# shubhamchandak94/HARC

Measured on AMD Instinct MI355X. Metric: Mreads/s reorder+encode, 100 bp, higher is better.
Workload: dtype u64 (2-bit packed bases, XOR+popcount)

## Files before the change

harc_amd/api.py:

```python
import ctypes as C
import os

HERE = os.path.dirname(os.path.abspath(__file__))


class HarcAmdError(RuntimeError):
    def __init__(self, code, msg):
        super().__init__(f"harc_amd error {code}: {msg}")
        self.code = code


class Params(C.Structure):
    _fields_ = [("readlen", C.c_int32), ("num_thr", C.c_int32), ("num_chains", C.c_int32), ("maxmatch", C.c_int32),
                ("thresh", C.c_int32), ("thresh_s", C.c_int32), ("maxsearch", C.c_int32), ("dict_start", C.c_int32 * 2),
                ("dict_end", C.c_int32 * 2), ("device", C.c_int32), ("profile", C.c_int32), ("num_steps", C.c_int32), ("reads_per_chain", C.c_int32), ("decode_memory_gb", C.c_int32), ("stream_digest", C.c_int32), ("table_slots_per_read", C.c_int32)]


class Counters(C.Structure):
    _fields_ = [("n_clean", C.c_uint64), ("n_N", C.c_uint64), ("n_main", C.c_uint64), ("n_singleton", C.c_uint64),
                ("unmatched", C.c_uint64), ("aligned_singletons", C.c_uint64), ("aligned_N", C.c_uint64),
                ("chains", C.c_uint64), ("rounds", C.c_uint64), ("probes", C.c_uint64), ("candidates", C.c_uint64),
                ("conflicts", C.c_uint64), ("propose_launches", C.c_uint64), ("propose_ms", C.c_double),
                ("index_ms", C.c_double), ("chain_ms", C.c_double), ("encode_ms", C.c_double), ("total_ms", C.c_double),
                ("contigs", C.c_uint64), ("seq_bases", C.c_uint64), ("bins_over_maxsearch", C.c_uint64),
# ... 48 lines not shown
    l.harc_amd_set_reads_ascii.argtypes = [ctx, C.c_char_p, C.c_uint32, C.c_uint32]
    l.harc_amd_set_reads_ascii_device.argtypes = [ctx, C.c_void_p, C.c_uint32, C.c_uint32]
    l.harc_amd_set_reads_packed_device.argtypes = [ctx, C.c_void_p, C.c_uint32]
    l.harc_amd_set_nreads_ascii.argtypes = [ctx, C.c_char_p, C.c_uint32, C.c_uint32]
    l.harc_amd_set_nreads_ascii_device.argtypes = [ctx, C.c_void_p, C.c_uint32, C.c_uint32]
    l.harc_amd_set_stage1_streams.argtypes = [ctx, C.c_char_p, C.c_char_p, C.c_char_p, C.c_char_p, C.c_char_p, C.c_uint32,
                                              C.c_char_p, C.c_char_p, C.c_uint32]
    l.harc_amd_pack_reads_device.argtypes = [ctx, C.c_void_p, C.c_uint32, C.c_uint32, C.c_void_p]
    l.harc_amd_bucket_reads_device.argtypes = [ctx, C.c_void_p, C.c_uint32, C.c_uint32, C.c_void_p]
    l.harc_amd_partition_reads_device.argtypes = [ctx, C.c_void_p, C.c_uint32, C.c_uint32, C.c_void_p, C.c_void_p]
    for f in ("harc_amd_reorder", "harc_amd_encode", "harc_amd_pack_order"):
        getattr(l, f).argtypes = [ctx]
    l.harc_amd_get_stream.argtypes = [ctx, C.c_int32, C.c_int32, C.POINTER(C.c_void_p), C.POINTER(C.c_size_t)]
    l.harc_amd_get_counters.argtypes = [ctx, C.POINTER(Counters)]
    for f in ("harc_amd_reorder_files", "harc_amd_encoder_files", "harc_amd_compress_files", "harc_amd_pack_order_files"):
        getattr(l, f).argtypes = [PP, C.c_char_p]
    l.harc_amd_preprocess_files.argtypes = [C.c_char_p, C.c_char_p, C.c_int32]
    l.harc_amd_decoder_files.argtypes = [PP, C.c_char_p, C.c_int32]
    l.harc_amd_compress_fastq_files_ex.argtypes = [PP, C.c_char_p, C.c_char_p, C.c_int32, C.c_int32]
    l.harc_amd_build_has.argtypes = [C.c_char_p]
    l.harc_amd_last_fastq_timing.argtypes = [C.POINTER(C.c_double), C.c_int32]
    l.harc_amd_decoder_preserve_files.argtypes = [PP, C.c_char_p, C.c_int32]
    l.harc_amd_compress_fastq_files.argtypes = [PP, C.c_char_p, C.c_char_p]
    l.harc_amd_set_fastq_device.argtypes = [ctx, C.c_void_p, C.c_uint64, C.POINTER(C.c_uint64)]
    l.harc_amd_bgzf_inflate_device.argtypes = [ctx, C.c_void_p, C.c_uint64, C.c_void_p, C.c_uint64, C.POINTER(C.c_uint64)]
    l.harc_amd_set_fastq_bgzf_device.argtypes = [ctx, C.c_void_p, C.c_uint64, C.POINTER(C.c_uint64)]
    l.harc_amd_fastq_assemble_device.argtypes = [ctx, C.c_void_p, C.c_uint64, C.c_void_p, C.c_void_p, C.c_uint32, C.c_int32, C.c_void_p, C.c_uint64,
                                                 C.POINTER(C.c_uint64)]
    l.harc_amd_fastq_assemble_files.argtypes = [PP, C.c_char_p, C.c_char_p, C.c_char_p, C.c_char_p]
    l.harc_amd_fastq_assemble_files_ex.argtypes = [PP, C.c_char_p, C.c_char_p, C.c_char_p, C.c_char_p, C.c_int32]
    l.harc_amd_bgzf_bound.argtypes = [C.c_uint64]
    l.harc_amd_bgzf_bound.restype = C.c_uint64
    l.harc_amd_bgzf_deflate_device.argtypes = [ctx, C.c_void_p, C.c_uint64, C.c_int32, C.c_void_p, C.c_uint64, C.POINTER(C.c_uint64)]
    l.harc_amd_bgzf_deflate_host.argtypes = [C.c_char_p, C.c_uint64, C.c_int32, C.c_char_p, C.c_uint64, C.POINTER(C.c_uint64)]
    l.harc_amd_qpack_bound.argtypes = [C.c_uint64, C.c_int32, C.c_uint32]
    l.harc_amd_qpack_bound.restype = C.c_uint64
    l.harc_amd_qpack_device.argtypes = [ctx, C.c_void_p, C.c_uint64, C.c_int32, C.c_uint32, C.c_int32, C.c_void_p, C.c_uint64, C.POINTER(C.c_uint64)]
    l.harc_amd_qunpack_device.argtypes = [ctx, C.c_void_p, C.c_uint64, C.c_void_p, C.c_uint64, C.POINTER(C.c_uint64)]
    l.harc_amd_qpack_host.argtypes = [C.c_char_p, C.c_uint64, C.c_int32, C.c_uint32, C.c_int32, C.c_char_p, C.c_uint64, C.POINTER(C.c_uint64)]
    l.harc_amd_qunpack_host.argtypes = [C.c_char_p, C.c_uint64, C.c_char_p, C.c_uint64, C.POINTER(C.c_uint64)]
    l.harc_amd_qpack_files.argtypes = [PP, C.c_char_p, C.c_char_p]
    l.harc_amd_qunpack_files.argtypes = [PP, C.c_char_p, C.c_char_p]
    QM, QS = C.POINTER(QMap), C.POINTER(QMapStats)
    l.harc_amd_qmap_parse.argtypes = [C.c_char_p, QM]
    l.harc_amd_qmap_host.argtypes = [C.c_char_p, C.c_uint64, C.c_int32, QM, C.c_char_p, QS]
    l.harc_amd_qmap_device.argtypes = [ctx, C.c_void_p, C.c_uint64, C.c_int32, QM, C.c_void_p, QS]
    l.harc_amd_qmap_files.argtypes = [PP, C.c_char_p, C.c_char_p, QM, QS]
    l.harc_amd_qpack_files_ex.argtypes = [PP, C.c_char_p, C.c_char_p, QM, QS]
    l.harc_amd_idpack_bound.argtypes = [C.c_uint64, C.c_uint64, C.c_uint32]
    l.harc_amd_idpack_bound.restype = C.c_uint64
    l.harc_amd_idpack_device.argtypes = [ctx, C.c_void_p, C.c_uint64, C.c_uint32, C.c_int32, C.c_void_p, C.c_uint64, C.POINTER(C.c_uint64)]
    l.harc_amd_idunpack_device.argtypes = [ctx, C.c_void_p, C.c_uint64, C.c_void_p, C.c_uint64, C.POINTER(C.c_uint64)]
    l.harc_amd_idpack_host.argtypes = [C.c_char_p, C.c_uint64, C.c_uint32, C.c_int32, C.c_char_p, C.c_uint64, C.POINTER(C.c_uint64)]
    l.harc_amd_idunpack_host.argtypes = [C.c_char_p, C.c_uint64, C.c_char_p, C.c_uint64, C.POINTER(C.c_uint64)]
    l.harc_amd_idpack_files.argtypes = [PP, C.c_char_p, C.c_char_p]
    l.harc_amd_idunpack_files.argtypes = [PP, C.c_char_p, C.c_char_p]
    l.harc_amd_spack_bound.argtypes = [C.c_uint64, C.c_uint32]
    l.harc_amd_spack_bound.restype = C.c_uint64
    l.harc_amd_spack_device.argtypes = [ctx, C.c_void_p, C.c_uint64, C.c_uint32, C.c_int32, C.c_void_p, C.c_uint64, C.POINTER(C.c_uint64)]
    l.harc_amd_sunpack_device.argtypes = [ctx, C.c_void_p, C.c_uint64, C.c_void_p, C.c_uint64, C.POINTER(C.c_uint64)]
    l.harc_amd_spack_host.argtypes = [C.c_char_p, C.c_uint64, C.c_uint32, C.c_int32, C.c_char_p, C.c_uint64, C.POINTER(C.c_uint64)]
    l.harc_amd_sunpack_host.argtypes = [C.c_char_p, C.c_uint64, C.c_char_p, C.c_uint64, C.POINTER(C.c_uint64)]
    l.harc_amd_spack_files.argtypes = [PP, C.c_char_p, C.c_char_p]
    l.harc_amd_sunpack_files.argtypes = [PP, C.c_char_p, C.c_char_p]
    l.harc_amd_spack_file_list.argtypes = [PP, C.c_int32, C.POINTER(C.c_char_p), C.POINTER(C.c_char_p)]
    l.harc_amd_sunpack_file_list.argtypes = [PP, C.c_int32, C.POINTER(C.c_char_p), C.POINTER(C.c_char_p)]
    l.harc_amd_decode_signature.argtypes = [ctx, C.POINTER(C.c_uint64)]
    l.harc_amd_input_signature.argtypes = [ctx, C.POINTER(C.c_uint64)]
    l.harc_amd_reads_signature_device.argtypes = [ctx, C.c_void_p, C.c_uint32, C.c_uint32, C.POINTER(C.c_uint64)]
    l.harc_amd_comm_get_id.argtypes = [C.c_char_p, C.c_size_t]
    l.harc_amd_comm_init.argtypes = [ctx, C.c_char_p, C.c_size_t, C.c_int32, C.c_int32]
    l.harc_amd_comm_init_mailbox.argtypes = [ctx, C.c_char_p, C.c_int32, C.c_int32]
    l.harc_amd_comm_barrier.argtypes = [ctx]
    l.harc_amd_comm_destroy.argtypes = [ctx]
    l.harc_amd_shard_exchange.argtypes = [ctx, C.POINTER(C.c_uint64)]
    l.harc_amd_shard_reset.argtypes = [ctx]
    l.harc_amd_replicate_exchange.argtypes = [ctx, C.POINTER(C.c_uint64)]
    l.harc_amd_compress_fastq_shard_files.argtypes = [PP, C.c_char_p, C.c_char_p, C.c_int32, C.c_int32, C.c_int32, C.c_int32, C.c_char_p]
    l.harc_amd_merge_shard_files.argtypes = [C.c_char_p, C.c_int32]
    l.harc_amd_stream_digest.argtypes = [ctx, C.POINTER(C.c_uint64)]
    l.harc_amd_selftest_launch.argtypes = [ctx, C.c_uint64, C.POINTER(C.c_uint64), C.POINTER(C.c_uint64)]
    l.harc_amd_selftest_index.argtypes = [ctx, C.c_void_p, C.c_uint64, C.c_int32, C.c_uint32, C.c_int32, C.POINTER(C.c_uint64), C.POINTER(C.c_uint32), C.c_void_p, C.c_void_p,
                                          C.c_void_p, C.c_uint64, C.POINTER(C.c_uint64)]
    U3 = C.POINTER(C.c_uint64)
    l.harc_amd_text_digest_device.argtypes = [ctx, C.c_void_p, C.c_uint64, C.c_uint64, U3]
    l.harc_amd_text_digest_host.argtypes = [C.c_char_p, C.c_uint64, C.c_uint64, U3]
    l.harc_amd_text_digest_files.argtypes = [PP, C.c_char_p, U3]
    l.harc_amd_input_order_digest.argtypes = [ctx, U3]
    l.harc_amd_reads_check_files.argtypes = [PP, C.c_char_p, U3, U3]
    l.harc_amd_compress_fastq_files_checked.argtypes = [PP, C.c_char_p, C.c_char_p, C.c_int32, C.c_int32, C.c_int32]
    l.harc_amd_build_id.restype = C.c_char_p
    _lib = l
    return l


def _check(rc):
    if rc != 0:
        raise HarcAmdError(rc, lib().harc_amd_last_error().decode(errors="replace"))


def default_params(readlen, num_thr=8, num_chains=0, device=0, profile=0, num_steps=0, reads_per_chain=0, stream_digest=0, table_slots_per_read=0):
    p = Params()
    _check(lib().harc_amd_default_params(readlen, C.byref(p)))
    p.num_thr, p.num_chains, p.device, p.profile, p.num_steps = num_thr, num_chains, device, profile, num_steps
    p.reads_per_chain = reads_per_chain
    p.stream_digest = stream_digest
    p.table_slots_per_read = table_slots_per_read
    return p


def build_id():
    return lib().harc_amd_build_id().decode()


def reorder(basedir, readlen, num_chains=1, **kw):
    p = default_params(readlen, num_chains=num_chains, **kw)
    _check(lib().harc_amd_reorder_files(C.byref(p), os.fsencode(basedir)))


def encoder(basedir, readlen, num_thr=1, **kw):
    p = default_params(readlen, num_thr=num_thr, **kw)
    _check(lib().harc_amd_encoder_files(C.byref(p), os.fsencode(basedir)))


def compress(basedir, readlen, num_thr=1, num_chains=1, **kw):
    p = default_params(readlen, num_thr=num_thr, num_chains=num_chains, **kw)
    _check(lib().harc_amd_compress_files(C.byref(p), os.fsencode(basedir)))


def preprocess(fastq, basedir, readlen):
    _check(lib().harc_amd_preprocess_files(os.fsencode(fastq), os.fsencode(basedir), readlen))


def compress_fastq(fastq, basedir, readlen, num_thr=1, num_chains=1, preserve_order=False, preserve_quality=False, check=False, **kw):
    p = default_params(readlen, num_thr=num_thr, num_chains=num_chains, **kw)
    _check(lib().harc_amd_compress_fastq_files_checked(C.byref(p), os.fsencode(fastq), os.fsencode(basedir), int(preserve_order), int(preserve_quality), int(check)))


def build_has(feature):
    return bool(lib().harc_amd_build_has(feature.encode()))


def last_fastq_timing(n=8):
    t = (C.c_double * n)()
    _check(lib().harc_amd_last_fastq_timing(t, n))
    names = ("context_and_pool", "ingest", "ingest_waiting_for_file_readers", "ingest_device_passes", "reorder", "encode", "stream_files", "total",
             "ingest_bgzf_inflate")
    return {k: float(v) for k, v in zip(names, t)}


COMM_ID_BYTES = 128


def comm_get_id():
    b = C.create_string_buffer(COMM_ID_BYTES)
    _check(lib().harc_amd_comm_get_id(b, COMM_ID_BYTES))
    return b.raw


def compress_fastq_shard(fastq, basedir, readlen, world, rank, comm_spec, num_thr=1, num_chains=0, preserve_order=False,
                         preserve_quality=False, **kw):
    kw.setdefault("reads_per_chain", 1024)
    p = default_params(readlen, num_thr=num_thr, num_chains=num_chains, **kw)
    _check(lib().harc_amd_compress_fastq_shard_files(C.byref(p), os.fsencode(fastq), os.fsencode(basedir), int(preserve_order),
                                                     int(preserve_quality), world, rank, os.fsencode(comm_spec)))

# ... 312 lines not shown
        _check(lib().harc_amd_comm_init(self._ctx, comm_id, len(comm_id), world, rank))

    def comm_init_mailbox(self, directory, world, rank):
        _check(lib().harc_amd_comm_init_mailbox(self._ctx, os.fsencode(directory), world, rank))

    def comm_barrier(self):
        _check(lib().harc_amd_comm_barrier(self._ctx))

    def comm_destroy(self):
        _check(lib().harc_amd_comm_destroy(self._ctx))

    def shard_exchange(self):
        info = (C.c_uint64 * 8)()
        _check(lib().harc_amd_shard_exchange(self._ctx, info))
        return tuple(int(x) for x in info)

    def replicate_exchange(self):
        info = (C.c_uint64 * 8)()
        _check(lib().harc_amd_replicate_exchange(self._ctx, info))
        return tuple(int(x) for x in info)

    def shard_reset(self):
        _check(lib().harc_amd_shard_reset(self._ctx))

    def reorder(self):
        _check(lib().harc_amd_reorder(self._ctx))

    def encode(self):
        _check(lib().harc_amd_encode(self._ctx))

    def pack_order(self):
        _check(lib().harc_amd_pack_order(self._ctx))

    def decode_signature(self):
        sig = (C.c_uint64 * 3)()
        _check(lib().harc_amd_decode_signature(self._ctx, sig))
        return tuple(int(x) for x in sig)

    def input_signature(self):
        sig = (C.c_uint64 * 3)()
        _check(lib().harc_amd_input_signature(self._ctx, sig))
        return tuple(int(x) for x in sig)

    def text_digest_device(self, ptr, nbytes, first_offset=0, acc=(0, 0, 0)):
        a = (C.c_uint64 * 3)(*acc)
        _check(lib().harc_amd_text_digest_device(self._ctx, C.c_void_p(ptr) if ptr else None, nbytes, first_offset, a))
        return tuple(a)

    def input_order_digest(self):
        a = (C.c_uint64 * 3)()
        _check(lib().harc_amd_input_order_digest(self._ctx, a))
        return tuple(a)

    def reads_signature_device(self, d_ascii, n, stride):
        sig = (C.c_uint64 * 3)()
        _check(lib().harc_amd_reads_signature_device(self._ctx, C.c_void_p(d_ascii), n, stride, sig))
        return tuple(int(x) for x in sig)

    def stream(self, name, shard=0):
        ptr, ln = C.c_void_p(), C.c_size_t()
        _check(lib().harc_amd_get_stream(self._ctx, STREAMS[name], shard, C.byref(ptr), C.byref(ln)))
        return C.string_at(ptr, ln.value) if ln.value else b""

    def selftest_launch(self, n):
        v, x = C.c_uint64(0), C.c_uint64(0)
        _check(lib().harc_amd_selftest_launch(self._ctx, n, C.byref(v), C.byref(x)))
        return int(v.value), int(x.value)

    def selftest_index(self, keys, slots_per_read=0, bigthresh=0, want_large=False):
        import numpy as np
        keys = np.ascontiguousarray(keys, dtype=np.uint64)
        n = int(keys.size)
        cap, nbins, nl = C.c_uint64(0), C.c_uint32(0), C.c_uint64(0)
        _check(lib().harc_amd_selftest_index(self._ctx, keys.ctypes.data, n, slots_per_read, bigthresh, 0, C.byref(cap), None, None, None, None, 0, None))
        slots = np.zeros(cap.value, dtype=np.dtype([("key", "<u8"), ("start", "<u4"), ("count", "<u4")]))
        ids = np.zeros(n, dtype=np.uint32)
        large = np.zeros(n // 16 + 16, dtype=np.uint64)
        _check(lib().harc_amd_selftest_index(self._ctx, keys.ctypes.data, n, slots_per_read, bigthresh, 1 if want_large else 0, C.byref(cap), C.byref(nbins),
                                             slots.ctypes.data, ids.ctypes.data, large.ctypes.data, large.size, C.byref(nl)))
        if want_large and nl.value > large.size:
            raise HarcAmdError(-1, "harc_amd_selftest_index lists %d large bins among %d keys" % (nl.value, n))
        return int(cap.value), int(nbins.value), slots, ids, (large[:nl.value].copy() if want_large else None)

    def stream_digest(self):
        d = (C.c_uint64 * 4)()
        _check(lib().harc_amd_stream_digest(self._ctx, d))
        return tuple(int(x) for x in d)

    def counters(self):
        c = Counters()
        _check(lib().harc_amd_get_counters(self._ctx, C.byref(c)))
        return c
```

harc_amd/csrc/api.cpp:

```cpp
#include "internal.h"
#include <stdarg.h>
#include <chrono>
#include <stdlib.h>

static thread_local char g_err[512] = "";
void harc_set_error(const char *fmt, ...)
{
    va_list ap; va_start(ap, fmt); vsnprintf(g_err, sizeof g_err, fmt, ap); va_end(ap);
}
extern "C" const char *harc_amd_last_error(void) { return g_err; }

static size_t pool_hand_back(harc_amd_ctx *c, size_t from, size_t asked)
{
    size_t given = 0;
    for (size_t i = 0; i < c->pool.size(); i++) {
        harc_amd_ctx::PoolChunk &k = c->pool[i];
        if (i == from || k.size == 0 || k.used != 0) continue;
        (void)hipFree(k.base); c->pool_total -= k.size; given += k.size; k.base = nullptr; k.size = 0;
    }
    if (given) {
        (void)hipGetLastError();
        if (getenv("HARC_AMD_TRACE")) fprintf(stderr, "[pool] %.2f GB of empty chunks handed back for a request of %.2f GB\n", given / 1e9, asked / 1e9);
    }
    return given;
}
int harc_raw_alloc(harc_amd_ctx *c, void **p, size_t bytes)
{
    *p = nullptr;
    if (bytes == 0) bytes = 16;
    hipError_t e = hipMalloc(p, bytes);
    if (e != hipSuccess) (void)hipGetLastError();
    if (e != hipSuccess && !c->pool.empty() && pool_hand_back(c, c->pool_cur, bytes)) e = hipMalloc(p, bytes);
    if (e != hipSuccess) { (void)hipGetLastError(); harc_set_error("hipMalloc(%zu) failed: %s", bytes, hipGetErrorString(e)); return HARC_AMD_ENOMEM; }
    c->owned.push_back(*p);
    c->sizes[*p] = bytes;
    c->dev_bytes += bytes;
    if (c->dev_bytes > c->dev_peak) c->dev_peak = c->dev_bytes;
    return HARC_AMD_OK;
}
void harc_raw_free(harc_amd_ctx *c, void *p)
{
    if (!p) return;
    for (size_t i = 0; i < c->owned.size(); i++)
        if (c->owned[i] == p) { c->owned[i] = c->owned.back(); c->owned.pop_back(); break; }
    auto it = c->sizes.find(p);
    if (it != c->sizes.end()) { c->dev_bytes -= it->second; c->sizes.erase(it); }
    (void)hipFree(p);
}
static size_t pool_in_use(const harc_amd_ctx *c)
{
    size_t u = 0;
    for (size_t i = 0; i <= c->pool_cur && i < c->pool.size(); i++) u += c->pool[i].used;
    return u;
}
int harc_dev_alloc(harc_amd_ctx *c, void **p, size_t bytes)
{
    *p = nullptr;
    if (const char *e = getenv("HARC_AMD_FAIL_ALLOC")) {
        static long long countdown = -1;
        if (countdown < 0) countdown = atoll(e);
        if (countdown > 0 && --countdown == 0) { harc_set_error("pool allocation refused (HARC_AMD_FAIL_ALLOC)"); return HARC_AMD_ENOMEM; }
    }
    bytes = (bytes + 255) & ~(size_t)255;
    if (bytes == 0) bytes = 256;
    const size_t cur_in = c->pool_cur;
    for (;;) {
        if (c->pool_cur < c->pool.size()) {
            harc_amd_ctx::PoolChunk &k = c->pool[c->pool_cur];
            if (k.used + bytes <= k.size) { *p = k.base + k.used; k.used += bytes; break; }
            if (c->pool_cur + 1 < c->pool.size()) { c->pool_cur++; c->pool[c->pool_cur].used = 0; continue; }
        }
        size_t want = bytes;
        const size_t grow = c->pool_total < ((size_t)8 << 30) ? c->pool_total : ((size_t)8 << 30);
        if (want < grow / 2) want = grow;
        if (want < ((size_t)64 << 20)) want = (size_t)64 << 20;
        void *base = nullptr;
        hipError_t e = hipMalloc(&base, want);
        if (e != hipSuccess) (void)hipGetLastError();
        if (e != hipSuccess && want > bytes) { want = bytes; e = hipMalloc(&base, want); if (e != hipSuccess) (void)hipGetLastError(); }
        if (e != hipSuccess && !c->pool.empty() && pool_hand_back(c, cur_in, bytes)) e = hipMalloc(&base, want);
        if (e != hipSuccess) { (void)hipGetLastError(); harc_set_error("hipMalloc(%zu) failed: %s", want, hipGetErrorString(e)); return HARC_AMD_ENOMEM; }
        if (getenv("HARC_AMD_POISON")) (void)hipMemset(base, 0xA5, want);
        if (getenv("HARC_AMD_TRACE")) fprintf(stderr, "[pool] chunk %zu: %.2f GB for a request of %.2f GB (pool %.2f GB, in use %.2f GB)\n", c->pool.size(), want / 1e9, bytes / 1e9, (c->pool_total + want) / 1e9, pool_in_use(c) / 1e9);
        c->pool.push_back({ (char *)base, want, 0 });
        c->pool_total += want;
        c->pool_cur = c->pool.size() - 1;
    }
    const size_t live = c->dev_bytes + pool_in_use(c);
    if (live > c->dev_peak) c->dev_peak = live;
    return HARC_AMD_OK;
}
void harc_dev_free(harc_amd_ctx *c, void *p) { (void)c; (void)p; }
harc_mark_t harc_pool_mark(harc_amd_ctx *c)
{
    if (c->pool.empty()) return 0;
    return ((harc_mark_t)c->pool_cur << 48) | (harc_mark_t)c->pool[c->pool_cur].used;
}
void harc_pool_release(harc_amd_ctx *c, harc_mark_t m)
{
    if (c->pool.empty()) return;
    const size_t cur = (size_t)(m >> 48), used = (size_t)(m & (((harc_mark_t)1 << 48) - 1));
    for (size_t i = cur + 1; i < c->pool.size(); i++) c->pool[i].used = 0;
    c->pool[cur].used = used;
    c->pool_cur = cur;
}
int harc_host_alloc(harc_amd_ctx *c, void **p, size_t bytes)
{
    bytes = (bytes + 63) & ~(size_t)63;
    if (bytes == 0) bytes = 64;
    for (auto &k : c->harena) if (k.used + bytes <= k.size) { *p = k.base + k.used; k.used += bytes; return HARC_AMD_OK; }
    size_t want = bytes < ((size_t)16 << 20) ? ((size_t)16 << 20) : bytes + (bytes >> 2);
    void *base = nullptr;
    hipError_t e = hipHostMalloc(&base, want, hipHostMallocDefault);
    if (e != hipSuccess) { harc_set_error("hipHostMalloc(%zu) failed: %s", want, hipGetErrorString(e)); return HARC_AMD_ENOMEM; }
    c->harena.push_back({ (char *)base, want, bytes });
    *p = base;
    return HARC_AMD_OK;
}
void harc_host_reset(harc_amd_ctx *c) { for (auto &k : c->harena) k.used = 0; }
int harc_d2h(harc_amd_ctx *c, std::vector<uint8_t> &dst, const void *d_src, size_t bytes)
{
    dst.resize(bytes);
    if (bytes) HIP_TRY(hipMemcpyAsync(dst.data(), d_src, bytes, hipMemcpyDeviceToHost, c->stream));
    return HARC_AMD_OK;
}

extern "C" int harc_amd_default_params(int32_t L, harc_amd_params *p)
{
    if (!p || L < 1 || L > 255) { harc_set_error("readlen %d out of range 1..255 (harc:46-49; 256 breaks the pos byte, decoder.cpp:93)", L); return HARC_AMD_EINVAL; }
    memset(p, 0, sizeof *p);
    p->readlen = L; p->num_thr = 8; p->num_chains = 0;
    p->maxmatch = L / 2; p->thresh = 4; p->thresh_s = 24; p->maxsearch = 1000;
    const int h = L / 2;
    if (L > 100) { p->dict_start[0] = h - 32; p->dict_end[0] = h - 1; p->dict_start[1] = h; p->dict_end[1] = h - 1 + 32; }
    else { p->dict_start[0] = h - L * 32 / 100; p->dict_end[0] = h - 1; p->dict_start[1] = h; p->dict_end[1] = h - 1 + L * 32 / 100; }
    return HARC_AMD_OK;
}

static int check_params(const harc_amd_params *p)
{
    if (!p) return HARC_AMD_EINVAL;
    const int L = p->readlen;
    if (L < 1 || L > 255) { harc_set_error("readlen %d out of range 1..255", L); return HARC_AMD_EINVAL; }
    if (p->num_thr < 1 || p->num_thr > 4096) { harc_set_error("num_thr %d out of range", p->num_thr); return HARC_AMD_EINVAL; }
    if (p->num_chains < 0) { harc_set_error("num_chains < 0"); return HARC_AMD_EINVAL; }
    if (p->num_steps < 0 || p->num_steps > 64) { harc_set_error("num_steps %d out of range 0..64", p->num_steps); return HARC_AMD_EINVAL; }
    if (p->maxmatch < 0 || p->maxmatch > 128 || p->maxmatch > L) { harc_set_error("maxmatch out of range"); return HARC_AMD_EINVAL; }
    if (p->maxsearch < 1 || p->thresh < 0 || p->thresh_s < 0) { harc_set_error("thresholds out of range"); return HARC_AMD_EINVAL; }
    for (int l = 0; l < 2; l++) {
        const int n = p->dict_end[l] - p->dict_start[l] + 1;
        if (p->dict_start[l] < 0 || p->dict_end[l] >= L || n < 0 || n > 32) { harc_set_error("dictionary window %d out of range", l); return HARC_AMD_EINVAL; }
    }
    return HARC_AMD_OK;
}

extern "C" int harc_amd_create(const harc_amd_params *params, harc_amd_ctx **out)
{
    if (!out) return HARC_AMD_EINVAL;
    *out = nullptr;
    RC_TRY(check_params(params));
    int ndev = 0;
    hipError_t e = hipGetDeviceCount(&ndev);
    if (e != hipSuccess || ndev <= 0) { harc_set_error("no HIP device (%s); libharc_amd has no CPU fallback", e == hipSuccess ? "count=0" : hipGetErrorString(e)); return HARC_AMD_ENODEVICE; }
    if (params->device < 0 || params->device >= ndev) { harc_set_error("device %d not in [0,%d)", params->device, ndev); return HARC_AMD_EINVAL; }
    HIP_TRY(hipSetDevice(params->device));
    harc_amd_ctx *c = new harc_amd_ctx();
    c->P = *params;
    c->W = (2 * params->readlen + 63) / 64;
    c->W3 = (3 * params->readlen + 63) / 64;
    memset(&c->C, 0, sizeof c->C);
    if (hipStreamCreateWithFlags(&c->stream, hipStreamNonBlocking) != hipSuccess) { delete c; harc_set_error("hipStreamCreate failed"); return HARC_AMD_ENODEVICE; }
    if (hipStreamCreateWithFlags(&c->copy_stream, hipStreamNonBlocking) != hipSuccess || hipEventCreateWithFlags(&c->ev_copy, hipEventDisableTiming) != hipSuccess) {
        if (c->copy_stream) (void)hipStreamDestroy(c->copy_stream);
        (void)hipStreamDestroy(c->stream); delete c; harc_set_error("hipStreamCreate failed"); return HARC_AMD_ENODEVICE;
    }
// ... 312 lines not shown
```

harc_amd/csrc/internal.h:

```cpp
#pragma once
#include <hip/hip_runtime.h>
#include <stdint.h>
#include <stdio.h>
#include <string.h>
#include <map>
#include <string>
#include <utility>
#include <vector>
#include "../../include/harc_amd.h"

#define HARC_NONE 0xFFFFFFFFu
#define HARC_MAXW 8
#define HARC_MAXW3 12
#define HARC_MAXK (1u << 20)
#define HARC_LOOK_CHUNKS 16
#ifndef HARC_NSUGG
#define HARC_NSUGG 8
#endif

void harc_set_error(const char *fmt, ...);

#define HIP_TRY(expr)                                                                                          \
    do {                                                                                                       \
        hipError_t _e = (expr);                                                                                \
// ... 38 lines not shown
};
#define SLOT_DEAD 0x80000000u
#define SLOT_EMB 0x40000000u
#define SLOT_BIG 0x20000000u
#define SLOT_OVF 0x10000000u
#define SLOT_CNT_MASK 0x0FFFFFFFu

struct DictDev {
    HashSlot *slots = nullptr;
    uint64_t cap = 0;
    uint32_t *ids = nullptr;
    uint32_t *d_nbins = nullptr;
    uint32_t nbins = 0;
    unsigned long long *large_list = nullptr; unsigned int *large_n = nullptr; uint32_t large_max = 0, large_tag = 0;
    uint32_t bigthresh = 0;
};

struct harc_amd_ctx {
    harc_amd_params P;
    int W = 0, W3 = 0;
    hipStream_t stream = nullptr;
    hipStream_t copy_stream = nullptr;
    hipEvent_t ev_copy = nullptr;
    uint32_t s2_events_hint = 0;
    uint64_t s1_seq_key = 0; int s1_seq_choice = -1;
    size_t dev_bytes = 0, dev_peak = 0;
    std::vector<void *> owned;
    std::map<void *, size_t> sizes;
    struct PoolChunk { char *base; size_t size, used; };
    std::vector<PoolChunk> pool;
    size_t pool_cur = 0, pool_total = 0;

    uint32_t N = 0;  uint64_t *d_reads = nullptr;
    uint32_t NN = 0; uint64_t *d_nreads3 = nullptr;
    struct InBuf { void *p = nullptr; size_t cap = 0; };
    InBuf own_reads, own_nreads3;
    uint32_t N_own = 0, NN_own = 0;
    uint64_t nrec_own = 0;
    struct HarcComm *comm = nullptr;
    InBuf x_reads, x_nreads3, x_gid, x_ngid;
    uint32_t *d_gid = nullptr, *d_ngid = nullptr;
    int s2_world = 1, s2_rank = 0;
    bool s2_part = false; int s2_e0 = 0, s2_e1 = 0;
    bool replicated = false;
    uint64_t shard_info[8] = { 0, 0, 0, 0, 0, 0, 0, 0 };
    bool have_s1 = false;
    uint32_t M = 0, S = 0;
    uint32_t *d_order = nullptr; uint8_t *d_flag = nullptr, *d_pos = nullptr, *d_rc = nullptr; uint32_t *d_order_s = nullptr;
    uint64_t *d_oreads = nullptr;
    uint64_t *d_sreads = nullptr;
    bool s1_from_files = false;
    bool have_s2 = false;
    uint32_t *d_s2_order = nullptr, *d_s2_orderN = nullptr; size_t n_s2_order = 0, n_s2_orderN = 0;

    struct OutBuf { const uint8_t *ptr = nullptr; size_t len = 0; std::vector<uint8_t> own; };
    std::map<std::pair<int, int>, OutBuf> out;
    struct HostChunk { char *base; size_t size, used; };
    std::vector<HostChunk> harena;
    harc_amd_counters C;
    uint64_t digest[4] = { 0, 0, 0, 0 }; bool have_digest = false;

    char *feed_ring = nullptr; size_t feed_ring_bytes = 0;

    void *d_tmp = nullptr; size_t tmp_bytes = 0;
};

struct HarcComm {
    int world = 1, rank = 0;
    virtual ~HarcComm() {}
    virtual int allgather_u64(harc_amd_ctx *c, const uint64_t *in, int n, uint64_t *out) = 0;
    virtual int alltoallv(harc_amd_ctx *c, int narr, const void *const *send, const size_t *const *soff, const size_t *const *sbytes,
                          void *const *recv, const size_t *const *roff, const size_t *const *rbytes) = 0;
    virtual int allreduce_min_u64(harc_amd_ctx *c, unsigned long long *d_buf, size_t n) = 0;
    virtual int wait(harc_amd_ctx *c, const char *what) = 0;
    virtual const char *name() const = 0;
};
int harc_in_reserve(harc_amd_ctx *c, harc_amd_ctx::InBuf *b, size_t bytes);
void harc_reset_shard(harc_amd_ctx *c);
void harc_drop_results(harc_amd_ctx *c);

int harc_dev_alloc(harc_amd_ctx *c, void **p, size_t bytes);
void harc_dev_free(harc_amd_ctx *c, void *p);
template <class T> static inline int dalloc(harc_amd_ctx *c, T **p, size_t n) { return harc_dev_alloc(c, (void **)p, n * sizeof(T) + 16); }
int harc_tmp_reserve(harc_amd_ctx *c, size_t bytes);
int harc_raw_alloc(harc_amd_ctx *c, void **p, size_t bytes);
void harc_raw_free(harc_amd_ctx *c, void *p);
typedef unsigned long long harc_mark_t;
harc_mark_t harc_pool_mark(harc_amd_ctx *c);
void harc_pool_release(harc_amd_ctx *c, harc_mark_t m);
struct PoolScope {
    harc_amd_ctx *c; harc_mark_t mk; bool armed = true;
    explicit PoolScope(harc_amd_ctx *c_) : c(c_), mk(harc_pool_mark(c_)) {}
    PoolScope(const PoolScope &) = delete;
    PoolScope &operator=(const PoolScope &) = delete;
    ~PoolScope() { if (armed) harc_pool_release(c, mk); }
    void keep() { armed = false; }
    void release_now() { if (armed) { harc_pool_release(c, mk); armed = false; } }
};

struct QmAcc;
int harc_qmap_check(const char *who, const harc_amd_qmap *map);
int harc_qmap_run(harc_amd_ctx *c, const char *d_text, uint64_t n, uint32_t L, const harc_amd_qmap *map, char *d_out, QmAcc *acc, double *seconds);

int prim_sort_pairs_u64_u32(harc_amd_ctx *c, const uint64_t *kin, uint64_t *kout, const uint32_t *vin, uint32_t *vout, size_t n, unsigned end_bit);
#define BL_TILE_WORDS 16384u
#define BL_PART_BITS 20
#define harc_bitmap_tiles(nwords) ((uint32_t)(((uint64_t)(nwords) + BL_TILE_WORDS - 1) / BL_TILE_WORDS))
#define harc_bitmap_item(w, b0, b1) (((uint64_t)((((uint32_t)(w) % BL_TILE_WORDS) << 10) | ((uint32_t)(b0) << 5) | (uint32_t)(b1)) << BL_PART_BITS) | (uint64_t)((uint32_t)(w) / BL_TILE_WORDS))
int harc_bitmap_from_items(harc_amd_ctx *c, const uint64_t *items, uint64_t *tmp, size_t n, uint64_t nwords, uint32_t *bitmap);
int prim_sort_keys_u64(harc_amd_ctx *c, const uint64_t *kin, uint64_t *kout, size_t n, unsigned end_bit);
int prim_excl_scan_u32(harc_amd_ctx *c, const uint32_t *in, uint32_t *out, size_t n);
int prim_excl_scan_u32_to_u64(harc_amd_ctx *c, const uint32_t *in, uint64_t *out, size_t n);
int prim_excl_scan_u8_to_u64(harc_amd_ctx *c, const uint8_t *in, uint64_t *out, size_t n);
int prim_incl_scan_u64(harc_amd_ctx *c, const uint64_t *in, uint64_t *out, size_t n);
int prim_incl_max_u32(harc_amd_ctx *c, const uint32_t *in, uint32_t *out, size_t n);
int prim_bins_scan(harc_amd_ctx *c, const uint64_t *skeys, size_t n, uint64_t cap, uint32_t *binstart, uint64_t *q, uint32_t *nbins, void *scratch, size_t scratch_bytes);

int s1_pack_ascii(harc_amd_ctx *c, const char *d_ascii, uint32_t n, uint32_t stride, uint64_t *d_out);
int s1_pack3_ascii(harc_amd_ctx *c, const char *d_ascii, uint32_t n, uint32_t stride, uint64_t *d_out);
int s1_unpack_to_ascii(harc_amd_ctx *c, const uint64_t *d_reads, uint32_t n, char *d_out);
int s1_bucket_reads(harc_amd_ctx *c, const uint64_t *d_packed, uint32_t n, uint32_t nb, uint32_t *d_out);
int s1_partition_reads(harc_amd_ctx *c, const uint64_t *d_packed, uint32_t n, uint32_t nb, uint64_t *d_out, unsigned long long *d_counts);
int shard_partition(harc_amd_ctx *c, const uint64_t *d_words, uint32_t n, int nwords, bool three_bit, uint32_t nb, uint32_t gid0,
                    uint64_t *d_out, uint32_t *d_gid_out, unsigned long long *d_counts);
int shard_map_ids(harc_amd_ctx *c, uint32_t *d_v, uint64_t n, const uint32_t *d_map, uint32_t nmap, unsigned int *d_err);
int stage1_run(harc_amd_ctx *c);
int stage1_make_oriented(harc_amd_ctx *c, uint32_t i0 = 0, uint32_t i1 = 0xFFFFFFFFu);
int s1_orient(harc_amd_ctx *c, const uint64_t *reads, const uint32_t *order, const uint8_t *rc, uint32_t m, uint64_t *out);
int harc_dict_alloc(harc_amd_ctx *c, DictDev *d, uint32_t n, uint64_t cap_like);
enum { HARC_KEYS_RAW = 0, HARC_KEYS_SORTABLE = 1 };
unsigned harc_dict_sort_bits(uint32_t n);
int harc_dict_build(harc_amd_ctx *c, DictDev *d, uint64_t *keys, uint32_t *ids, uint32_t n, unsigned kbits, int keys_are);
void harc_dict_free(harc_amd_ctx *c, DictDev *d);
int stage2_run(harc_amd_ctx *c);
int pack_order_run(harc_amd_ctx *c);

static inline std::vector<uint8_t> &out_buf(harc_amd_ctx *c, int id, int shard) { harc_amd_ctx::OutBuf &o = c->out[std::make_pair(id, shard)]; o.ptr = nullptr; o.len = 0; return o.own; }
static inline void out_slice(harc_amd_ctx *c, int id, int shard, const void *p, size_t n) { harc_amd_ctx::OutBuf &o = c->out[std::make_pair(id, shard)]; o.own.clear(); o.ptr = (const uint8_t *)p; o.len = n; }
int harc_host_alloc(harc_amd_ctx *c, void **p, size_t bytes);
void harc_host_reset(harc_amd_ctx *c);
int harc_d2h(harc_amd_ctx *c, std::vector<uint8_t> &dst, const void *d_src, size_t bytes);

int build_line_index(harc_amd_ctx *c, const char *d_txt, uint64_t nbytes, const uint64_t **nls_out, uint64_t *total_lines_out);

int write_shard_family(harc_amd_ctx *c, const std::string &od, int first_shard, int e_lo = 0, int e_hi = -1);
int write_whole_job_files(harc_amd_ctx *c, const std::string &od);

struct BgzfCand { uint64_t off; uint32_t bsize, hdr, isize, crc; };
struct BgzfMember { uint64_t cdata, text; uint32_t clen, isize, crc, hdr; };
struct BgzfPlan { std::vector<BgzfMember> m; uint64_t text = 0, next = 0; };
int harc_bgzf_plan(harc_amd_ctx *c, const uint8_t *d_in, uint64_t n, uint64_t start, uint64_t own_end, uint64_t base_off, BgzfPlan *plan);
int harc_bgzf_run(harc_amd_ctx *c, const uint8_t *d_in, const BgzfPlan &plan, uint64_t base_off, char *d_out);

struct BgzfOutStats { uint64_t text = 0, bytes = 0, members = 0, stored = 0; double seconds = 0; };
int harc_bgzf_deflate(harc_amd_ctx *c, const char *d_text, uint64_t n_bytes, int32_t flags, uint8_t *d_out, uint64_t out_capacity, uint64_t *n_out, BgzfOutStats *st);
```

harc_amd/csrc/prims.hip:

```cpp
#include "devutil.h"
#include <rocprim/rocprim.hpp>

int harc_tmp_reserve(harc_amd_ctx *c, size_t bytes)
{
    if (bytes <= c->tmp_bytes) return HARC_AMD_OK;
    if (c->d_tmp) harc_raw_free(c, c->d_tmp);
    c->d_tmp = nullptr; c->tmp_bytes = 0;
    size_t want = bytes + (bytes >> 3) + 4096;
    RC_TRY(harc_raw_alloc(c, &c->d_tmp, want));
    c->tmp_bytes = want;
    return HARC_AMD_OK;
}

#define PRIM_CALL(call_with_tmp)                                \
    do {                                                        \
        size_t bytes = 0; void *tmp = nullptr;                  \
        HIP_TRY(call_with_tmp);                                 \
        RC_TRY(harc_tmp_reserve(c, bytes));                     \
        tmp = c->d_tmp; bytes = c->tmp_bytes;                   \
        HIP_TRY(call_with_tmp);                                 \
    } while (0)

int prim_sort_pairs_u64_u32(harc_amd_ctx *c, const uint64_t *kin, uint64_t *kout, const uint32_t *vin, uint32_t *vout, size_t n, unsigned end_bit)
{
// ... 37 lines not shown
    PRIM_CALL(rocprim::exclusive_scan(tmp, bytes, it, out, (uint64_t)0, n, rocprim::plus<uint64_t>(), c->stream));
    return HARC_AMD_OK;
}

int prim_incl_scan_u64(harc_amd_ctx *c, const uint64_t *in, uint64_t *out, size_t n)
{
    if (n == 0) return HARC_AMD_OK;
    PRIM_CALL(rocprim::inclusive_scan(tmp, bytes, in, out, n, rocprim::plus<uint64_t>(), c->stream));
    return HARC_AMD_OK;
}

int prim_incl_max_u32(harc_amd_ctx *c, const uint32_t *in, uint32_t *out, size_t n)
{
    if (n == 0) return HARC_AMD_OK;
    PRIM_CALL(rocprim::inclusive_scan(tmp, bytes, in, out, n, rocprim::maximum<uint32_t>(), c->stream));
    return HARC_AMD_OK;
}

struct BinPart { long long m; uint32_t c, pad; };
struct BinPartOp {
    __host__ __device__ BinPart operator()(const BinPart &a, const BinPart &b) const
    {
        const long long bm = b.m - (long long)a.c;
        return BinPart{ a.m > bm ? a.m : bm, a.c + b.c, 0u };
    }
};
#define BINS_NONE (-(1ll << 62))
#define BINS_SEG_MIN 2048u
#define BINS_UNROLL 4
template <bool WRITE> __global__ __launch_bounds__(256) void k_bins_pass(const uint64_t *k, uint32_t n, uint64_t cap, uint32_t seg, uint32_t nseg, BinPart *part,
                                                                       uint32_t *binstart, uint64_t *q, uint32_t *nbins)
{
    const uint32_t w = (blockIdx.x * 256u + threadIdx.x) >> 6;
    if (w >= nseg) return;
    const int lane = threadIdx.x & 63;
    const unsigned long long below = ((unsigned long long)1 << lane) - 1;
    uint32_t C = 0; long long M = BINS_NONE;
    if (WRITE) { C = part[w].c; M = part[w].m; }
    const uint64_t base = (uint64_t)w * seg, end = base + seg < n ? base + seg : (uint64_t)n;
    uint64_t carry = base ? k[base - 1] : 0;
    for (uint64_t at = base; at < end; at += 64u * BINS_UNROLL) {
        uint64_t key[BINS_UNROLL];
#pragma unroll
        for (int u = 0; u < BINS_UNROLL; u++) { const uint64_t i = at + 64u * u + lane; key[u] = i < end ? k[i] : 0; }
#pragma unroll
        for (int u = 0; u < BINS_UNROLL; u++) {
            const uint64_t i = at + 64u * u + lane;
            uint64_t prev = __shfl_up(key[u], 1, 64);
            if (lane == 0) prev = carry;
            carry = __shfl(key[u], 63, 64);
            const bool head = i < end && (i == 0 || key[u] != prev);
            const unsigned long long hb = __ballot(head);
            const uint32_t rank = C + (uint32_t)__popcll(hb & below);
            long long v = head ? (long long)bucket_slot(key[u], cap) - (long long)rank : BINS_NONE;
            if (WRITE) {
                for (int d = 1; d < 64; d <<= 1) { const long long o = __shfl_up(v, d, 64); if (lane >= d && o > v) v = o; }
                if (M > v) v = M;
                if (head) { binstart[rank] = (uint32_t)i; q[rank] = (uint64_t)(v + (long long)n); }
                if (i < end && i + 1 == n) *nbins = rank + (head ? 1u : 0u);
                M = __shfl(v, 63, 64);
            } else if (v > M) M = v;
            C += (uint32_t)__popcll(hb);
        }
    }
    if (!WRITE) {
        for (int o = 32; o > 0; o >>= 1) { const long long x = __shfl_xor(M, o, 64); if (x > M) M = x; }
        if (lane == 0) part[w] = BinPart{ M, C, 0u };
    }
}
int prim_bins_scan(harc_amd_ctx *c, const uint64_t *skeys, size_t n, uint64_t cap, uint32_t *binstart, uint64_t *q, uint32_t *nbins, void *scratch, size_t scratch_bytes)
{
    if (n == 0) return HARC_AMD_OK;
    const size_t room = scratch_bytes / (2 * sizeof(BinPart));
    if (room == 0 || n > 0xFFFFFFFFull || (n + room - 1) / room > (1u << 30) || room > 0x7FFFFFFFull) { harc_set_error("prim_bins_scan: %zu keys, scratch of %zu bytes", n, scratch_bytes); return HARC_AMD_EINVAL; }
    size_t seg = (n + room - 1) / room;
    if (seg < BINS_SEG_MIN) seg = BINS_SEG_MIN;
    seg = (seg + 64 * BINS_UNROLL - 1) / (64 * BINS_UNROLL) * (64 * BINS_UNROLL);
    const uint32_t nseg = (uint32_t)((n + seg - 1) / seg);
    BinPart *part = (BinPart *)scratch, *front = part + nseg;
    const dim3 grid((nseg + 3) / 4);
    hipLaunchKernelGGL(k_bins_pass<false>, grid, dim3(256), 0, c->stream, skeys, (uint32_t)n, cap, (uint32_t)seg, nseg, part, (uint32_t *)nullptr, (uint64_t *)nullptr, (uint32_t *)nullptr);
    PRIM_CALL(rocprim::exclusive_scan(tmp, bytes, part, front, BinPart{ BINS_NONE, 0u, 0u }, (size_t)nseg, BinPartOp(), c->stream));
    hipLaunchKernelGGL(k_bins_pass<true>, grid, dim3(256), 0, c->stream, skeys, (uint32_t)n, cap, (uint32_t)seg, nseg, front, binstart, q, nbins);
    HIP_TRY(hipGetLastError());
    return HARC_AMD_OK;
}

__global__ void k_selftest_grid(uint64_t n, unsigned long long *out)
{
    const uint64_t i = harc_gid();
    unsigned long long one = i < n ? 1ULL : 0ULL, idx = i < n ? (unsigned long long)i : 0ULL;
    for (int o = 32; o > 0; o >>= 1) { one += __shfl_xor(one, o, 64); idx += __shfl_xor(idx, o, 64); }
    if ((threadIdx.x & 63) == 0 && one) { atomicAdd(&out[0], one); atomicAdd(&out[1], idx); }
}
__global__ void k_selftest_grid32(uint32_t n, unsigned long long *out)
{
    const uint32_t i = harc_gid32();
    unsigned long long one = i < n ? 1ULL : 0ULL, idx = i < n ? (unsigned long long)i : 0ULL;
    for (int o = 32; o > 0; o >>= 1) { one += __shfl_xor(one, o, 64); idx += __shfl_xor(idx, o, 64); }
    if ((threadIdx.x & 63) == 0 && one) { atomicAdd(&out[0], one); atomicAdd(&out[1], idx); }
}
__global__ void k_selftest_fold(uint64_t n, unsigned long long *out)
{
    const uint64_t wave = harc_bid() * 4 + (threadIdx.x >> 6);
    const int lane = threadIdx.x & 63;
    const uint64_t i = wave * 16 + (uint64_t)(lane >> 2);
    const bool mine = i < n && (lane & 3) == 0;
    unsigned long long one = mine ? 1ULL : 0ULL, idx = mine ? (unsigned long long)i : 0ULL;
    for (int o = 32; o > 0; o >>= 1) { one += __shfl_xor(one, o, 64); idx += __shfl_xor(idx, o, 64); }
    if (lane == 0 && one) { atomicAdd(&out[0], one); atomicAdd(&out[1], idx); }
}
extern "C" int harc_amd_selftest_launch(harc_amd_ctx *c, uint64_t n, uint64_t *visited, uint64_t *index_sum)
{
    if (!c || !visited || !index_sum) return HARC_AMD_EINVAL;
    HIP_TRY(hipSetDevice(c->P.device));
    unsigned long long *d = nullptr, h[6] = { 0, 0, 0, 0, 0, 0 };
    HIP_TRY(hipMalloc((void **)&d, sizeof h));
    const bool n32 = n <= 0xFFFFFFFFull;
    hipError_t e = hipMemsetAsync(d, 0, sizeof h, c->stream);
    if (e == hipSuccess) { hipLaunchKernelGGL(k_selftest_grid, harc_grid256(n), dim3(256), 0, c->stream, n, d); e = hipGetLastError(); }
    if (e == hipSuccess && n32) { hipLaunchKernelGGL(k_selftest_grid32, harc_grid256(n), dim3(256), 0, c->stream, (uint32_t)n, d + 2); e = hipGetLastError(); }
    if (e == hipSuccess) { hipLaunchKernelGGL(k_selftest_fold, harc_fold256((n + 63) / 64), dim3(256), 0, c->stream, n, d + 4); e = hipGetLastError(); }
    if (e == hipSuccess) e = hipMemcpyAsync(h, d, sizeof h, hipMemcpyDeviceToHost, c->stream);
    if (e == hipSuccess) e = hipStreamSynchronize(c->stream);
    (void)hipFree(d);
    if (e != hipSuccess) { harc_set_error("harc_amd_selftest_launch: %s", hipGetErrorString(e)); return HARC_AMD_ENODEVICE; }
    int k = 0;
    if (n32 && (h[2] != h[0] || h[3] != h[1])) k = 2;
    else if (h[4] != h[0] || h[5] != h[1]) k = 4;
    if (k) harc_set_error("harc_amd_selftest_launch: %s visited %llu items (index sum %llx), the thread-per-item grid %llu (%llx)", k == 2 ? "harc_gid32" : "harc_fold256 / harc_bid", h[k], h[k + 1], h[0], h[1]);
    *visited = h[k]; *index_sum = h[k + 1];
    return k ? HARC_AMD_EINTERNAL : HARC_AMD_OK;
}
```

harc_amd/csrc/stage2.hip:

```cpp
#include "devutil.h"
#include <time.h>
#include <algorithm>
#include <stdlib.h>

#define TUPLE_NONE 0xFFFFFFFFFFFFFFFFULL

struct S2Args {
    int L, W, W3, thresh_s, maxsearch;
    int ds[2], de[2], kbits[2];
    uint32_t M, S, T, q, nC;
    uint64_t total;
    const uint64_t *oreads;
    const uint8_t *flag, *pos, *rc;
    const uint32_t *order;
    const uint64_t *cand3;
    const uint32_t *cand_order;
    uint8_t *head;
    uint64_t *gstart;
    uint8_t *cons;
    const uint32_t *chead;
    const HashSlot *slots[2]; uint64_t cap[2]; const uint32_t *ids[2];
    unsigned long long *best;
    unsigned long long *bestbin[2];
    const uint32_t *bloom[2]; int bloom_shift[2];
    int bloom_lbits, bloom_nwin;
    const uint64_t *cons2;
    const uint64_t *cand2, *candN;
    uint4 *events;
    unsigned int *nevents; uint32_t maxevents;
    int trace;
    uint64_t col0, col1; uint32_t tile_base;
    const uint64_t *evwin;
    unsigned long long *cbb[2]; uint32_t *cpos[2], *ccnt[2]; unsigned long long *tminbin[2]; int compact;
    int binmax_on;
    unsigned long long *binmax[2];
};

__device__ __forceinline__ int base2_at(const uint64_t *r, int j) { return (int)((r[j >> 5] >> (2 * (j & 31))) & 3); }
__device__ __forceinline__ int pc_to_idx(int pc) { return ((pc & 1) << 1) | (pc >> 1); }
__device__ __forceinline__ int c3_at(const uint64_t *r, int W3, int j)
{
    const int off = 3 * j, wi = off >> 6, sh = off & 63;
    uint64_t v = r[wi] >> sh;
    if (sh > 61 && wi + 1 < W3) v |= r[wi + 1] << (64 - sh);
    return (int)(v & 7);
}
__device__ __forceinline__ int c3_to_idx5(int c3) { return c3 == 0 ? 0 : c3 == 4 ? 1 : c3 == 2 ? 2 : c3 == 6 ? 3 : 4; }
__device__ __forceinline__ int idx_to_c3(int idx) { return idx == 0 ? 0 : idx == 1 ? 4 : idx == 2 ? 2 : 6; }
__device__ __forceinline__ int comp5(int b) { return b == 4 ? 4 : 3 - b; }
__device__ __forceinline__ char enc_noise(int ref, int rd)
{
    const unsigned tabA = 0x32100, tabC = 0x32100, tabG = 0x30021, tabT = 0x30012;
    const unsigned t = ref == 0 ? tabA : ref == 1 ? tabC : ref == 2 ? tabG : tabT;
    return (char)('0' + ((t >> (4 * rd)) & 0xF));
}
__device__ __forceinline__ long long ub_le(const uint64_t *a, long long n, uint64_t x)
{
    long long lo = -1, hi = n;
    while (hi - lo > 1) { const long long mid = (lo + hi) >> 1; if (a[mid] <= x) lo = mid; else hi = mid; }
    return lo;
}

__global__ void k_cand3_from2(const uint64_t *reads2, const uint32_t *gather, uint32_t n, int L, int W, int W3, uint64_t *out)
{
    const size_t gid = harc_gid();
    if (gid >= (size_t)n * W3) return;
    const uint32_t i = (uint32_t)(gid / W3); const int w = (int)(gid % W3);
    const uint64_t *r = reads2 + (size_t)(gather ? gather[i] : i) * W;
    uint64_t v = 0;
    const int b0 = (64 * w) / 3, b1 = (64 * w + 63) / 3;
    for (int b = b0; b <= b1 && b < L; b++) {
        const uint64_t c3 = (uint64_t)(2 * base2_at(r, b));
        const int sh = 3 * b - 64 * w;
        v |= sh >= 0 ? (c3 << sh) : (c3 >> (-sh));
    }
    out[gid] = v;
}
__global__ void k_cand_order(const uint32_t *order_s, uint32_t S, uint32_t T, uint32_t *out)
{
    const uint32_t i = harc_gid32();
    if (i >= T) return;
    out[i] = i < S ? order_s[i] : i - S;
}
__global__ void k_key3(const uint64_t *cand3, uint32_t T, int W3, int off, int nbits, uint64_t *keys, uint32_t *ids)
{
    const uint32_t i = harc_gid32();
    if (i >= T) return;
    const uint64_t *r = cand3 + (size_t)i * W3;
    const int wi = off >> 6, sh = off & 63;
    uint64_t v = r[wi] >> sh;
    if (sh && wi + 1 < W3) v |= r[wi + 1] << (64 - sh);
    if (nbits < 64) v &= ((uint64_t)1 << nbits) - 1;
    keys[i] = v; ids[i] = i;
}
__global__ void k_count_big_bins(const HashSlot *slots, uint64_t cap, uint32_t maxsearch, unsigned long long *out)
{
    const uint64_t i = harc_gid();
    if (i >= cap) return;
    if ((slots[i].count & SLOT_CNT_MASK) > maxsearch) atomicAdd(out, 1ULL);
}

__global__ void k_heads1(const uint8_t *flag, uint32_t M, uint32_t q, uint8_t *head, uint32_t *hidx)
{
    const uint32_t i = harc_gid32();
    if (i >= M) return;
    const uint8_t h = (flag[i] == '0' || (i % q) == 0) ? 1 : 0;
    head[i] = h; hidx[i] = h ? i : 0;
}
__global__ void k_heads2(uint32_t M, uint8_t *head, const uint32_t *hmax, uint32_t *hidx)
{
    const uint32_t i = harc_gid32();
    if (i >= M) return;
    const uint32_t r = i - hmax[i];
    if (r > 0 && (r % 10000001u) == 0) head[i] = 1;
    hidx[i] = head[i] ? 1u : 0u;
}
__global__ void k_col_steps(const uint8_t *head, const uint8_t *pos, uint32_t M, int L, uint64_t *d)
{
    const uint32_t i = harc_gid32();
    if (i >= M) return;
    d[i] = head[i] ? (i == 0 ? 0 : (uint64_t)L) : (uint64_t)pos[i];
}
__global__ void k_contig_heads(const uint8_t *head, const uint32_t *cid, uint32_t M, uint32_t *chead)
{
    const uint32_t i = harc_gid32();
    if (i >= M) return;
    if (head[i]) chead[cid[i]] = i;
}

__global__ void k_contig_info(S2Args s, unsigned long long *cinfo)
{
    const uint32_t k = harc_gid32();
    if (k >= s.nC) return;
    const bool lastc = (k + 1 == s.nC) || (s.chead[k + 1] % s.q) == 0;
    const unsigned long long cend = (k + 1 == s.nC) ? s.total : s.gstart[s.chead[k + 1]];
    cinfo[k] = cend | ((unsigned long long)lastc << 63);
}

#define CSTRIP 16
#define CTHREADS 128
#define CTILE (CTHREADS * CSTRIP)
#ifndef CCHUNK
#define CCHUNK 256
#endif
#ifndef CL0
#define CL0 4
#endif
#define CPLANES 32
#ifndef CSHALLOW
#define CSHALLOW 12
#endif
__global__ void k_consensus_tiles(S2Args s, uint32_t ntiles, uint32_t *tlo, uint32_t *thi)
{
    const uint32_t t = harc_gid32();
    if (t >= ntiles) return;
    const uint64_t X0 = (uint64_t)(t + s.tile_base) * CTILE, X1 = X0 + CTILE < s.total ? X0 + CTILE : s.total;
    thi[t] = (uint32_t)ub_le(s.gstart, (long long)s.M, X1 - 1);
    tlo[t] = X0 >= (uint64_t)s.L ? (uint32_t)(ub_le(s.gstart, (long long)s.M, X0 - (uint64_t)s.L) + 1) : 0u;
}
template <int NPL> __global__ __launch_bounds__(CTHREADS, NPL == CPLANES ? 4 : 6) void k_consensus(S2Args s, const uint32_t *cid, const unsigned long long *cinfo, int want_windows, const uint32_t *tlo, const uint32_t *thi, uint32_t *tovf)
{
    if (NPL == CPLANES && !tovf[blockIdx.x]) return;
    extern __shared__ uint64_t cl_words[];
    int *const cl_g = reinterpret_cast<int *>(cl_words + (size_t)CCHUNK * s.W);
    const uint32_t *const cl_w32 = reinterpret_cast<const uint32_t *>(cl_words);
    const uint64_t X0 = (uint64_t)(blockIdx.x + s.tile_base) * CTILE;
    const int L = s.L, W = s.W;
    const long long ilo = tlo[blockIdx.x], ihi = thi[blockIdx.x];
    const int x0r = (int)threadIdx.x * CSTRIP;
    const uint64_t x0 = X0 + (uint64_t)x0r;
    const bool mine = x0 < s.total;
    const int ncol = !mine ? 0 : x0 + CSTRIP <= s.total ? CSTRIP : (int)(s.total - x0);
    const int xlr = x0r + ncol - 1;
    const uint32_t EVEN = 0x55555555u;
    uint32_t lo[2][CL0], pl[2][NPL];
#pragma unroll
    for (int j = 0; j < CL0; j++) lo[0][j] = lo[1][j] = 0;
#pragma unroll
    for (int j = 0; j < NPL; j++) pl[0][j] = pl[1][j] = 0;
    bool ovf = false;
    int pend = 0, depth = CL0;
    auto flush = [&]() {
        uint32_t ca = 0, cb = 0;
#pragma unroll
        for (int j = 0; j < CL0; j++) {
            const uint32_t xa = pl[0][j] ^ lo[0][j], xb = pl[1][j] ^ lo[1][j];
            const uint32_t na = (pl[0][j] & lo[0][j]) | (xa & ca), nb = (pl[1][j] & lo[1][j]) | (xb & cb);
            pl[0][j] = xa ^ ca; pl[1][j] = xb ^ cb; ca = na; cb = nb;
            lo[0][j] = lo[1][j] = 0;
        }
#pragma unroll
        for (int j = CL0; j < CSHALLOW; j++) {
#ifndef HARC_CONS_FIXED_DEPTH
            if (__builtin_amdgcn_ballot_w64((ca | cb) != 0) == 0) break;
#endif
            const uint32_t ta = pl[0][j] & ca, tb = pl[1][j] & cb;
            pl[0][j] ^= ca; pl[1][j] ^= cb; ca = ta; cb = tb;
            if (depth < j + 1) depth = j + 1;
        }
        if (NPL > CSHALLOW) {
#ifndef HARC_CONS_FIXED_DEPTH
            if (__builtin_amdgcn_ballot_w64((ca | cb) != 0) != 0)
#endif
            {
#pragma unroll
                for (int j = CSHALLOW; j < NPL; j++) {
                    const uint32_t ta = pl[0][j] & ca, tb = pl[1][j] & cb;
                    pl[0][j] ^= ca; pl[1][j] ^= cb; ca = ta; cb = tb;
                }
                depth = NPL;
            }
        } else ovf |= (ca | cb) != 0;
        pend = 0;
    };
    long long ilast = ilo - 1;
    int nstart = 0;
    for (long long base = ilo; base <= ihi; base += CCHUNK) {
        const int nch = (int)(ihi + 1 - base < CCHUNK ? ihi + 1 - base : CCHUNK);
        __syncthreads();
        for (int k = threadIdx.x; k < nch * W; k += CTHREADS) cl_words[k] = s.oreads[(size_t)base * W + k];
        for (int k = threadIdx.x; k < nch; k += CTHREADS) cl_g[k] = (int)((long long)s.gstart[base + k] - (long long)X0);
        __syncthreads();
        int k = nch;
        if (mine) {
            int a = -1, b = nch;
            while (b - a > 1) { const int mid = (a + b) >> 1; if (cl_g[mid] <= x0r - L) a = mid; else b = mid; }
            k = b;
        }
        auto start_of = [&](int kk) { return kk < nch ? cl_g[kk] : 0x7FFFFFFF; };
        auto window_of = [&](int kk, int g, uint32_t &w0, uint32_t &w1) {
            const int o0 = x0r - g, j0 = o0 < 0 ? 0 : o0;
            const uint32_t *r = cl_w32 + (size_t)(kk < nch ? kk : nch - 1) * (2 * W) + (j0 >> 4);
            w0 = r[0]; w1 = r[1];
        };
        int g = start_of(k), gn = start_of(k + 1);
        uint32_t w0, w1;
        window_of(k, g, w0, w1);
        for (;; k++) {
            const bool act = g <= xlr;
            if (__builtin_amdgcn_ballot_w64(act) == 0) break;
            uint32_t w0n, w1n;
            window_of(k + 1, gn, w0n, w1n);
            const int gnn = start_of(k + 2);
            if (act) {
                if (g <= x0r) ilast = base + k; else nstart++;
                const int o0 = x0r - g;
                uint32_t bits = __builtin_amdgcn_alignbit(w1, w0, (uint32_t)(2 * ((o0 < 0 ? 0 : o0) & 15)));
                if (o0 < 0) bits <<= 2 * (-o0);
                const int c_lo = o0 < 0 ? -o0 : 0, c_hi = L - o0 < ncol ? L - o0 : ncol;
                uint32_t vm = c_hi >= CSTRIP ? 0xFFFFFFFFu : ((1u << (2 * (c_hi > 0 ? c_hi : 0))) - 1u);
                vm &= ~((1u << (2 * c_lo)) - 1u) & EVEN;
                const uint32_t b0 = bits & vm, b1 = (bits >> 1) & vm;
                uint32_t ma = (vm & ~(b0 | b1)) | ((b0 & ~b1) << 1);
                uint32_t mb = (b1 & ~b0) | ((b0 & b1) << 1);
#pragma unroll
                for (int j = 0; j < CL0; j++) {
                    const uint32_t ta = lo[0][j] & ma, tb = lo[1][j] & mb;
                    lo[0][j] ^= ma; lo[1][j] ^= mb; ma = ta; mb = tb;
                }
            }
            g = gn; gn = gnn; w0 = w0n; w1 = w1n;
            if (++pend == (1 << CL0) - 1) flush();
        }
    }
    flush();
    if (NPL < CPLANES && ovf) tovf[blockIdx.x] = 1;
    if (!mine) return;
    depth = __builtin_amdgcn_readfirstlane(depth);
    uint32_t lt = 0, dec = 0, lt2 = 0, dec2 = 0;
#pragma unroll
    for (int j = NPL - 1; j >= 0; j--)
        if (j < depth) { const uint32_t d = pl[0][j] ^ pl[1][j]; lt |= d & ~dec & pl[1][j]; dec |= d; }
#pragma unroll
    for (int j = NPL - 1; j >= 0; j--)
        if (j < depth) {
            const uint32_t w = (pl[0][j] & ~lt) | (pl[1][j] & lt), d = (w ^ (w >> 1)) & EVEN;
            lt2 |= d & ~dec2 & (w >> 1); dec2 |= d;
        }
    const uint32_t indw = (lt2 & (lt >> 1)) | (~lt2 & lt & EVEN) | (lt2 << 1);
    uint32_t outw[CSTRIP / 4];
    uint32_t vmask = 0;
    if (want_windows) {
        const long long ie = ilast + nstart;
        const uint32_t ka = cid[ilast] + (uint32_t)s.head[ilast] - 1u, ke = cid[ie] + (uint32_t)s.head[ie] - 1u;
        unsigned long long ci = cinfo[ka];
        if (ka == ke) {
            const unsigned long long cend = ci & ~(1ULL << 63);
            if (!(ci >> 63) && x0 + (uint64_t)L <= cend) { const unsigned long long nv = cend - (x0 + (uint64_t)L) + 1; vmask = nv >= CSTRIP ? 0xFFFFu : (1u << (int)nv) - 1u; }
        } else {
            uint32_t kprev = ka; long long i = ilast;
            uint64_t gnext = i + 1 < (long long)s.M ? s.gstart[i + 1] : ~0ull;
            bool moved = false;
            for (int c = 0; c < ncol; c++) {
                const uint64_t x = x0 + c;
                while (gnext <= x) { i++; gnext = i + 1 < (long long)s.M ? s.gstart[i + 1] : ~0ull; moved = true; }
                if (moved) {
                    const uint32_t k = cid[i] + (uint32_t)s.head[i] - 1u;
                    if (k != kprev) { ci = cinfo[k]; kprev = k; }
                    moved = false;
                }
                if (!(ci >> 63) && x + (uint64_t)L <= (ci & ~(1ULL << 63))) vmask |= 1u << c;
            }
        }
    }
#pragma unroll
    for (int c = 0; c < CSTRIP; c++) {
        if ((c & 3) == 0) outw[c >> 2] = 0;
        outw[c >> 2] |= (((indw >> (2 * c)) & 3u) | (((vmask >> c) & 1u) << 2)) << (8 * (c & 3));
    }
    if (ncol == CSTRIP) {
        *reinterpret_cast<uint4 *>(s.cons + x0) = make_uint4(outw[0], outw[1], outw[2], outw[3]);
    } else {
        for (int c = 0; c < ncol; c++) s.cons[x0 + c] = (uint8_t)(outw[c >> 2] >> (8 * (c & 3)));
    }
}

__device__ __forceinline__ bool dict_lookup_b(const HashSlot *tab, uint64_t cap, uint64_t key, uint32_t *start, uint32_t *count)
{
    key = key_scramble(key);
    uint64_t sl = bucket_slot(key, cap);
    for (;;) {
        const uint4 r0 = *reinterpret_cast<const uint4 *>(&tab[sl]), r1 = *reinterpret_cast<const uint4 *>(&tab[sl + 1]);
        if (r0.w == 0) return false;
        if (((uint64_t)r0.x | ((uint64_t)r0.y << 32)) == key) { *start = r0.z; *count = r0.w; return true; }
        if (r1.w == 0) return false;
        if (((uint64_t)r1.x | ((uint64_t)r1.y << 32)) == key) { *start = r1.z; *count = r1.w; return true; }
        const uint4 r2 = *reinterpret_cast<const uint4 *>(&tab[sl + 2]), r3 = *reinterpret_cast<const uint4 *>(&tab[sl + 3]);
        if (r2.w == 0) return false;
        if (((uint64_t)r2.x | ((uint64_t)r2.y << 32)) == key) { *start = r2.z; *count = r2.w; return true; }
        if (r3.w == 0) return false;
        if (((uint64_t)r3.x | ((uint64_t)r3.y << 32)) == key) { *start = r3.z; *count = r3.w; return true; }
        if (!(r0.w & SLOT_OVF)) return false;
        sl += 4; if (sl >= cap) sl = 0;
    }
}
__global__ void k_bloom_set(const uint64_t *keys, uint32_t n, uint32_t *bloom, int shift)
{
    const uint32_t i = harc_gid32();
    if (i >= n) return;
    const uint64_t b = mix64(keys[i] ^ 0x9E3779B97F4A7C15ULL) >> shift;
    atomicOr(&bloom[b >> 5], 1u << (b & 31));
}
#ifndef BLOOM4_M
#define BLOOM4_M 15
#endif
__device__ __forceinline__ uint32_t bloom4_mmer(uint64_t fk)
{
    const uint32_t h = ((uint32_t)fk & ((1u << (2 * BLOOM4_M)) - 1u)) * 0x9E3779B1u;
    return h ^ (h >> 15);
}
__device__ __forceinline__ uint32_t bloom4_minimizer(uint64_t fk, int nwin)
{
    uint32_t best = 0xFFFFFFFFu;
    for (int i = 0; i < nwin; i++) { const uint32_t x = bloom4_mmer(fk >> (2 * i)); best = x < best ? x : best; }
    return best;
}
__device__ __forceinline__ void bloom4_pos(uint64_t fk, uint32_t minz, int nwin, int lbits, uint32_t *word, int *sh0, int *sh1)
{
    uint32_t kh = ((uint32_t)fk * 0x9E3779B1u) ^ ((uint32_t)(fk >> 32) * 0x85EBCA77u);
    kh ^= kh >> 15; kh *= 0xC2B2AE3Du; kh ^= kh >> 13;
    uint32_t lh = nwin > 0 ? minz * 0x9E3779B1u : kh * 0x165667B1u;
    lh ^= lh >> 15; lh *= 0x85EBCA77u; lh ^= lh >> 13;
    *word = ((lh >> (32 - lbits)) << 4) | ((kh >> 6) & 15u);
    *sh0 = 4 * (int)(kh & 7u); *sh1 = 4 * (int)((kh >> 3) & 7u);
}
__global__ void k_bloom4_set(const uint64_t *keys, uint32_t n, uint32_t *bloom, int lbits, int nwin, int l, int nb)
{
    const uint32_t i = harc_gid32();
    if (i >= n) return;
    const uint64_t k = keys[i];
    uint64_t f = 0, r = 0;
    for (int b = 0; b < nb; b++) {
        const uint32_t c3 = (uint32_t)(k >> (3 * b)) & 7u;
        if (c3 & 1u) return;
        const uint64_t idx = ((c3 >> 2) & 1u) | (c3 & 2u);
        f |= idx << (2 * b); r |= (3u - idx) << (2 * (nb - 1 - b));
    }
    uint32_t w; int a, b;
    bloom4_pos(f, bloom4_minimizer(f, nwin), nwin, lbits, &w, &a, &b);
    atomicOr(&bloom[w], ((1u << l) << a) | ((1u << l) << b));
    bloom4_pos(r, bloom4_minimizer(r, nwin), nwin, lbits, &w, &a, &b);
    atomicOr(&bloom[w], ((4u << l) << a) | ((4u << l) << b));
}
__global__ void k_bloom4_items(const uint64_t *keys, uint32_t n, int lbits, int nwin, int l, int nb, uint32_t skip_tile, uint64_t *items)
{
    const uint32_t i = harc_gid32();
    if (i >= n) return;
    const uint64_t k = keys[i];
    uint64_t f = 0, r = 0; bool hasn = false;
    for (int b = 0; b < nb; b++) {
        const uint32_t c3 = (uint32_t)(k >> (3 * b)) & 7u;
        hasn |= (c3 & 1u) != 0;
        const uint64_t idx = ((c3 >> 2) & 1u) | (c3 & 2u);
        f |= idx << (2 * b); r |= (3u - idx) << (2 * (nb - 1 - b));
    }
    if (hasn) { items[2 * (size_t)i] = items[2 * (size_t)i + 1] = (uint64_t)skip_tile; return; }
// ... 673 lines not shown
    unsigned long long todo = __ballot(in);
    while (todo) {
        const int leader = __ffsll((long long)todo) - 1;
        const uint32_t lk = __shfl(k, leader, 64);
        const unsigned long long same = __ballot(in && k == lk);
        if ((threadIdx.x & 63) == leader) atomicAdd(&hist[lk], (unsigned int)__popcll(same));
        todo &= ~same;
    }
}
__global__ void k_ev_seglen(const uint32_t *rank, uint32_t nev, uint32_t *seglen)
{
    const uint32_t i = harc_gid32();
    if (i >= nev) return;
    if (i + 1 == nev || rank[i + 1] == 0) seglen[i - rank[i]] = rank[i] + 1;
}

__global__ void k_acc_flags(const unsigned long long *best, uint32_t T, uint32_t *flag)
{
    const uint32_t i = harc_gid32();
    if (i >= T) return;
    flag[i] = best[i] != TUPLE_NONE ? 1u : 0u;
}
__global__ void k_acc_compact(const unsigned long long *best, const uint32_t *rank, uint32_t T, uint32_t A, uint64_t *tup, uint32_t *rid)
{
    const uint32_t i = harc_gid32();
    if (i >= T) return;
    if (best[i] != TUPLE_NONE) { const uint32_t at = A - 1 - rank[i]; tup[at] = best[i]; rid[at] = i; }
}

struct FinalArrays { uint32_t *ref; uint8_t *kind; uint64_t *g; };
__global__ void k_merge_cuts(const uint64_t *gstart, uint32_t i0, uint32_t n, const uint64_t *tup, uint32_t A, long long *cut)
{
    const uint32_t b = harc_gid32(), nb = (n + 255u) / 256u;
    if (b > nb) return;
    const uint32_t t = b < nb ? b * 256u : n - 1u;
    const uint64_t g = gstart[i0 + t];
    long long lo = -1, hi = A;
    while (hi - lo > 1) { const long long mid = (lo + hi) >> 1; if ((tup[mid] >> 2) < g) lo = mid; else hi = mid; }
    cut[b] = lo;
}
#define MERGE_TILE 2048
__global__ __launch_bounds__(256) void k_merge_orig(const uint64_t *gstart, uint32_t i0, uint32_t n, const uint64_t *tup, uint32_t A, FinalArrays f, uint32_t fbase, const long long *cut)
{
    __shared__ uint64_t cols[MERGE_TILE];
    const uint32_t t = harc_gid32();
    const long long c0 = cut[harc_bid()], c1 = cut[harc_bid() + 1] + 1;
    const long long inside = c1 - c0 - 1;
    const bool tiled = inside <= MERGE_TILE;
    if (tiled) {
        for (long long j = threadIdx.x; j < inside; j += 256) cols[j] = tup[c0 + 1 + j] >> 2;
        __syncthreads();
    }
    if (t >= n) return;
    const uint32_t i = i0 + t;
    const uint64_t g = gstart[i];
    long long lo = c0, hi = c1;
    if (tiled) while (hi - lo > 1) { const long long mid = (lo + hi) >> 1; if (cols[mid - c0 - 1] < g) lo = mid; else hi = mid; }
    else while (hi - lo > 1) { const long long mid = (lo + hi) >> 1; if ((tup[mid] >> 2) < g) lo = mid; else hi = mid; }
    const uint32_t at = i + (uint32_t)(lo + 1) - fbase;
    f.ref[at] = i; f.kind[at] = 0; f.g[at] = g;
}
__global__ void k_merge_acc(const uint64_t *gstart, uint32_t M, const uint64_t *tup, const uint32_t *rid, uint32_t a0, uint32_t na, FinalArrays f, uint32_t fbase)
{
    const uint32_t t = harc_gid32();
    if (t >= na) return;
    const uint32_t k = a0 + t;
    const uint64_t x = tup[k] >> 2;
    const long long n = ub_le(gstart, (long long)M, x) + 1;
    const uint32_t at = k + (uint32_t)n - fbase;
    f.ref[at] = rid[k]; f.kind[at] = (tup[k] & 2) ? 2 : 1; f.g[at] = x;
}
__global__ void k_shard_bounds(const uint64_t *gstart, uint32_t M, uint32_t q, uint32_t E, const uint64_t *tup, uint32_t A, uint64_t total, uint32_t *sh_f, uint32_t *sh_a, uint64_t *sh_col)
{
    const uint32_t e = harc_gid32();
    if (e > E) return;
    const uint64_t st = (uint64_t)e * q;
    if (e == E || st >= M) { sh_f[e] = M + A; sh_a[e] = A; sh_col[e] = total; return; }
    const uint64_t g = gstart[st];
    long long lo = -1, hi = A;
    while (hi - lo > 1) { const long long mid = (lo + hi) >> 1; if ((tup[mid] >> 2) < g) lo = mid; else hi = mid; }
    sh_f[e] = (uint32_t)st + (uint32_t)(lo + 1); sh_a[e] = (uint32_t)(lo + 1); sh_col[e] = g;
}

__global__ void k_pack_cons2(const uint8_t *cons, uint64_t total, uint64_t w0, uint64_t nwords, uint64_t *cons2)
{
    const uint64_t w = w0 + harc_gid();
    if (w >= w0 + nwords) return;
    uint64_t v = 0;
    const uint64_t c0 = w * 32;
    if (c0 + 32 <= total) {
        const uint4 q0 = *(const uint4 *)(cons + c0), q1 = *(const uint4 *)(cons + c0 + 16);
        const uint32_t qq[8] = { q0.x, q0.y, q0.z, q0.w, q1.x, q1.y, q1.z, q1.w };
#pragma unroll
        for (int k = 0; k < 32; k++) { const uint32_t idx = (qq[k >> 2] >> (8 * (k & 3))) & 3; v |= (uint64_t)(((idx & 1) << 1) | (idx >> 1)) << (2 * k); }
    } else {
        for (int k = 0; k < 32 && c0 + k < total; k++) { const uint32_t idx = cons[c0 + k] & 3; v |= (uint64_t)(((idx & 1) << 1) | (idx >> 1)) << (2 * k); }
    }
    cons2[w] = v;
}
template <int W> __device__ __forceinline__ void final_words(const S2Args &s, uint32_t ref, int kind, uint64_t (&rd)[W], uint64_t (&nmk)[W])
{
    if (kind == 0) {
        const uint64_t *r = s.oreads + (size_t)ref * W;
#pragma unroll
        for (int w = 0; w < W; w++) { rd[w] = r[w]; nmk[w] = 0; }
        return;
    }
    constexpr int W3M = (3 * 32 * W + 63) / 64;
    uint64_t x3[W3M + 1];
    const uint64_t *r = s.cand3 + (size_t)ref * s.W3;
#pragma unroll
    for (int w = 0; w <= W3M; w++) x3[w] = w < s.W3 ? r[w] : 0;
    uint64_t a[W], n[W];
#pragma unroll
    for (int w = 0; w < W; w++) { a[w] = 0; n[w] = 0; }
#pragma unroll
    for (int j = 0; j < 32 * W; j++) {
        const int off = 3 * j, wi = off >> 6, sh = off & 63;
        uint64_t v = x3[wi] >> sh;
        if (sh > 61) v |= x3[wi + 1] << (64 - sh);
        const uint64_t c3 = v & 7;
        a[j >> 5] |= (c3 >> 1) << (2 * (j & 31));
        n[j >> 5] |= ((c3 & 1) * 3) << (2 * (j & 31));
    }
#pragma unroll
    for (int w = 0; w < W; w++) { const uint64_t lm = lowmask_word(2 * s.L, w); a[w] &= lm; n[w] &= lm; }
    if (kind == 1) {
#pragma unroll
        for (int w = 0; w < W; w++) { rd[w] = a[w]; nmk[w] = n[w]; }
    } else {
        uint64_t t[W];
        rc_words<W>(a, s.L, rd);
        rc_words<W>(n, s.L, t);
#pragma unroll
        for (int w = 0; w < W; w++) nmk[w] = ~t[w] & lowmask_word(2 * s.L, w);
    }
}
template <int W, bool EMIT> __global__ void k_noise(S2Args s, FinalArrays f, const uint64_t *cons2, uint32_t fb, uint32_t F, uint32_t *nm, uint32_t *nonN,
                                                    const uint64_t *nmoff, const uint32_t *nonNrank,
                                                    uint8_t *noise, uint8_t *noisepos, uint8_t *posb, uint8_t *rcb, uint32_t *order_out, uint32_t *orderN_out)
{
    const uint64_t i64 = (uint64_t)fb + harc_gid();
    if (i64 >= F) return;
    const uint32_t i = (uint32_t)i64;
    const uint32_t ref = f.ref[i]; const int kind = f.kind[i]; const uint64_t g = f.g[i];
    uint64_t rd[W], nk[W], cw[W], mm[W];
    final_words<W>(s, ref, kind, rd, nk);
    cons_words<W>(cons2, g, cw);
    uint32_t cnt = 0;
#pragma unroll
    for (int w = 0; w < W; w++) {
        const uint64_t x = rd[w] ^ cw[w];
        mm[w] = ((x | (x >> 1) | nk[w]) & 0x5555555555555555ULL) & lowmask_word(2 * s.L, w);
        cnt += (uint32_t)__popcll(mm[w]);
    }
    if (!EMIT) {
        nm[i] = cnt;
        nonN[i] = (kind != 0 && ref >= s.S) ? 0u : 1u;
        return;
    }
    uint64_t np = nmoff[i], nz = nmoff[i] + i;
    int prevj = 0;
#pragma unroll
    for (int w = 0; w < W; w++) {
        uint64_t m = mm[w];
        while (m) {
            const int b = __ffsll((long long)m) - 1; m &= m - 1;
            const int j = 32 * w + (b >> 1);
            const int rb = ((nk[w] >> b) & 1) ? 4 : pc_to_idx((int)((rd[w] >> b) & 3)), cb = pc_to_idx((int)((cw[w] >> b) & 3));
            noise[nz++] = (uint8_t)enc_noise(cb, rb); noisepos[np++] = (uint8_t)(j - prevj); prevj = j;
        }
    }
    noise[nz] = '\n';
    const bool is_head = (kind == 0) && s.head[ref];
    posb[i] = is_head ? (uint8_t)s.L : (uint8_t)(g - f.g[i - 1]);
    rcb[i] = kind == 0 ? s.rc[ref] : (kind == 1 ? 'd' : 'r');
    const uint32_t ov = kind == 0 ? s.order[ref] : s.cand_order[ref];
    const bool isN = (kind != 0 && ref >= s.S);
    if (isN) orderN_out[i - nonNrank[i]] = ov; else order_out[nonNrank[i]] = ov;
}
template <bool EMIT> static void launch_noise(harc_amd_ctx *c, const S2Args &a, const FinalArrays &f, const uint64_t *cons2, uint32_t fb, uint32_t F, uint32_t *nm, uint32_t *nonN,
                                              const uint64_t *nmoff, const uint32_t *nonNrank, uint8_t *noise, uint8_t *noisepos, uint8_t *posb, uint8_t *rcb,
                                              uint32_t *order_out, uint32_t *orderN_out)
{
#define NOISE_CASE(WW) case WW: hipLaunchKernelGGL((k_noise<WW, EMIT>), harc_grid256(F - fb), dim3(256), 0, c->stream, a, f, cons2, fb, F, nm, nonN, nmoff, nonNrank, noise, noisepos, posb, rcb, order_out, orderN_out); break;
    switch (a.W) { NOISE_CASE(1) NOISE_CASE(2) NOISE_CASE(3) NOISE_CASE(4) NOISE_CASE(5) NOISE_CASE(6) NOISE_CASE(7) NOISE_CASE(8) }
#undef NOISE_CASE
}

__global__ void k_left_flags(const unsigned long long *best, uint32_t t0, uint32_t n, uint32_t S, uint32_t *fs, uint32_t *fn)
{
    const uint32_t t = harc_gid32();
    if (t >= n) return;
    const uint32_t i = t0 + t;
    const bool un = best[i] == TUPLE_NONE;
    fs[t] = (un && i < S) ? 1u : 0u; fn[t] = (un && i >= S) ? 1u : 0u;
}
__global__ void k_left_orders(S2Args s, uint32_t t0, uint32_t nt, const uint32_t *rs, const uint32_t *rn, uint32_t *order_out, uint32_t order_base, uint32_t *orderN_out, uint32_t orderN_base)
{
    const uint32_t t = harc_gid32();
    if (t >= nt) return;
    const uint32_t i = t0 + t;
    if (s.best[i] != TUPLE_NONE) return;
    if (i < s.S) order_out[order_base + rs[t]] = s.cand_order[i]; else orderN_out[orderN_base + rn[t]] = s.cand_order[i];
}
__global__ void k_left_emit(S2Args s, uint32_t t0, uint32_t nt, const uint32_t *rs, const uint32_t *rn, uint8_t *sing_bases, char *ntext)
{
    const int G = (s.L + 15) / 16;
    const uint64_t gid = harc_gid();
    if (gid >= (uint64_t)nt * G) return;
    const uint32_t i = t0 + (uint32_t)(gid / G); const int g = (int)(gid % G);
    if (s.best[i] != TUPLE_NONE) return;
    const uint64_t *r = s.cand3 + (size_t)i * s.W3;
    const int j0 = 16 * g, j1 = j0 + 16 < s.L ? j0 + 16 : s.L;
    if (i < s.S) {
        const uint32_t k = rs[i - t0];
        uint8_t *o = sing_bases + (size_t)k * s.L;
        for (int j = j0; j < j1; j++) o[j] = (uint8_t)c3_to_idx5(c3_at(r, s.W3, j));
    } else {
        const uint32_t k = rn[i - t0];
        char *o = ntext + (size_t)k * (s.L + 1);
        for (int j = j0; j < j1; j++) o[j] = "ACGTN"[c3_to_idx5(c3_at(r, s.W3, j))];
        if (j1 == s.L) o[s.L] = '\n';
    }
}

__global__ void k_left_list(const uint32_t *fs, const uint32_t *fn, const uint32_t *rs, const uint32_t *rn, uint32_t nt, uint32_t US, uint32_t *list)
{
    const uint32_t t = harc_gid32();
    if (t >= nt) return;
    if (fs[t]) list[rs[t]] = t;
    else if (fn[t]) list[US + rn[t]] = t;
}
__global__ __launch_bounds__(256) void k_left_emit_w(S2Args s, uint32_t t0, const uint32_t *list, uint32_t nl, uint32_t US, uint8_t *sing_bases, char *ntext, uint32_t kbase)
{
    const uint32_t q = kbase + blockIdx.x * 4u + (threadIdx.x >> 6);
    const int lane = threadIdx.x & 63;
    if (q >= nl) return;
    const uint32_t i = t0 + list[q];
    const uint64_t *r = s.cand3 + (size_t)i * s.W3;
    const bool single = q < US;
    uint8_t *const ob = sing_bases + (size_t)q * s.L;
    char *const ot = ntext + (size_t)(q - US) * (s.L + 1);
    for (int j = lane; j < s.L; j += 64) {
        const int off = 3 * j, wi = off >> 6, sh = off & 63;
        const uint64_t lo = r[wi], hi = wi + 1 < s.W3 ? r[wi + 1] : 0ULL;
        const int c3 = (int)(((lo >> sh) | (sh ? (hi << (64 - sh)) : 0ULL)) & 7ULL);
        const int b = c3_to_idx5(c3);
        if (single) ob[j] = (uint8_t)b; else ot[j] = "ACGTN"[b];
    }
    if (!single && lane == 0) ot[s.L] = '\n';
}

__global__ void k_pack2_bytes(const uint8_t *bases, uint64_t nbytes_out, uint8_t *out)
{
    const uint64_t i = harc_gid();
    if (i >= nbytes_out) return;
    const uint8_t *b = bases + 4 * i;
    out[i] = (uint8_t)((b[0] & 3) | ((b[1] & 3) << 2) | ((b[2] & 3) << 4) | ((b[3] & 3) << 6));
}
__global__ void k_pack1_bytes(const uint8_t *rc, uint64_t nbytes_out, uint8_t *out)
{
    const uint64_t i = harc_gid();
    if (i >= nbytes_out) return;
    const uint8_t *b = rc + 8 * i;
    uint8_t v = 0;
    for (int k = 0; k < 8; k++) v |= (uint8_t)((b[k] == 'r') << k);
    out[i] = v;
}
__global__ void k_bases_to_ascii(const uint8_t *bases, uint64_t n, uint8_t *out)
{
    const uint64_t i = harc_gid();
    if (i >= n) return;
    out[i] = (uint8_t)"ACGT"[bases[i] & 3];
}

__global__ void k_pack_order(const uint32_t *order, uint32_t ngroups, int numbits, uint32_t *out)
{
    const uint64_t gid = harc_gid();
    if (gid >= (uint64_t)ngroups * numbits) return;
    const uint32_t g = (uint32_t)(gid / numbits); const int w = (int)(gid % numbits);
    const int k0 = (32 * w) / numbits, k1 = (32 * w + 31) / numbits;
    uint32_t v = 0;
    for (int k = k0; k <= k1 && k < 32; k++) {
        const uint32_t o = order[(size_t)g * 32 + k];
        const int sh = k * numbits - 32 * w;
        v |= sh >= 0 ? (o << sh) : (o >> (-sh));
    }
    out[gid] = v;
}

__global__ void k_stream_digest(const uint8_t *base, uint64_t nbytes, uint64_t salt, unsigned long long *out)
{
    const uint64_t nw = (nbytes + 7) / 8;
    unsigned long long acc = 0;
    for (uint64_t i = (uint64_t)blockIdx.x * blockDim.x + threadIdx.x; i < nw; i += (uint64_t)gridDim.x * blockDim.x) {
        uint64_t v = reinterpret_cast<const uint64_t *>(base)[i];
        const uint64_t left = nbytes - 8 * i;
        if (left < 8) v &= ((uint64_t)1 << (8 * left)) - 1;
        acc += mix64(v ^ mix64(i * 0x9E3779B97F4A7C15ULL + salt));
    }
    for (int o = 32; o > 0; o >>= 1) acc += __shfl_xor(acc, o, 64);
    if ((threadIdx.x & 63) == 0 && acc) atomicAdd(out, acc);
}

#define WAVE_PER_ITEM(n, launch) do { const uint64_t nwg_ = ((uint64_t)(n) + 3) / 4; for (uint64_t b_ = 0; b_ < nwg_; b_ += (1u << 23)) { \
        const unsigned nb_ = (unsigned)(nwg_ - b_ < (1u << 23) ? nwg_ - b_ : (1u << 23)); const uint32_t kb_ = (uint32_t)(b_ * 4); launch; } } while (0)
#define G256(n) harc_grid256((uint64_t)(n)), dim3(256), 0, c->stream
static int digest_range(harc_amd_ctx *c, const void *base, uint64_t nbytes, uint64_t salt, unsigned long long *d_out)
{
    if (!nbytes) return HARC_AMD_OK;
    if ((uintptr_t)base & 7) { harc_set_error("stream digest: a stream does not start on an 8-byte boundary"); return HARC_AMD_EINTERNAL; }
    const uint64_t nw = (nbytes + 7) / 8;
    const unsigned nb = (unsigned)(nw / 1024 + 1 < 4096 ? nw / 1024 + 1 : 4096);
    hipLaunchKernelGGL(k_stream_digest, dim3(nb), dim3(256), 0, c->stream, (const uint8_t *)base, nbytes, salt, d_out);
    HIP_TRY(hipGetLastError());
    return HARC_AMD_OK;
}

int stage2_run(harc_amd_ctx *c)
{
    const harc_amd_params &P = c->P;
    const int L = P.readlen, W = c->W, W3 = c->W3;
    const uint32_t M = c->M, S = c->S, NN = c->NN, T = S + NN, E = (uint32_t)P.num_thr;
    for (auto it = c->out.begin(); it != c->out.end();) { if (it->first.first >= HARC_AMD_S2_SEQ) it = c->out.erase(it); else ++it; }
    const bool part = c->s2_part;
    HarcComm *const cm = (part && c->comm && c->replicated) ? c->comm : nullptr;
    const uint32_t pw = part ? (uint32_t)c->s2_world : 1u, pr = part ? (uint32_t)c->s2_rank : 0u;
    const uint32_t e0 = part ? (uint32_t)c->s2_e0 : 0u, e1 = part ? (uint32_t)c->s2_e1 : E;
    const uint32_t t0 = (uint32_t)((uint64_t)T * pr / pw), t1 = (uint32_t)((uint64_t)T * (pr + 1u) / pw);
    const bool trace2 = getenv("HARC_AMD_TRACE") != nullptr;
    struct timespec tl0; clock_gettime(CLOCK_MONOTONIC, &tl0);
    auto lap = [&](const char *what) { if (trace2) { (void)hipStreamSynchronize(c->stream); struct timespec t; clock_gettime(CLOCK_MONOTONIC, &t); fprintf(stderr, "[stage II%s] %s: %.1f ms\n", part ? " (partitioned)" : "", what, (t.tv_sec - tl0.tv_sec) * 1e3 + (t.tv_nsec - tl0.tv_nsec) * 1e-6); tl0 = t; } };

    S2Args a; memset(&a, 0, sizeof a);
    a.L = L; a.W = W; a.W3 = W3; a.thresh_s = P.thresh_s; a.maxsearch = P.maxsearch;
    if (L > 50) { a.ds[0] = 0; a.de[0] = 20; a.ds[1] = 21; a.de[1] = 41; }
    else { a.ds[0] = 0; a.de[0] = 20 * L / 50; a.ds[1] = 20 * L / 50 + 1; a.de[1] = 41 * L / 50; }
    for (int l = 0; l < 2; l++) a.kbits[l] = 3 * (a.de[l] - a.ds[l] + 1);
    a.M = M; a.S = S; a.T = T;
    a.q = 1u + (uint32_t)((M - 1u) / E);
    if (a.q == 0) a.q = 1;
    a.oreads = c->d_oreads; a.flag = c->d_flag; a.pos = c->d_pos; a.rc = c->d_rc; a.order = c->d_order;
    const uint32_t i0 = (uint32_t)((uint64_t)e0 * a.q > M ? M : (uint64_t)e0 * a.q), i1 = e1 >= E ? M : (uint32_t)((uint64_t)e1 * a.q > M ? M : (uint64_t)e1 * a.q);

    uint32_t *order_out = nullptr, *orderN_out = nullptr;
    RC_TRY(dalloc(c, &order_out, (size_t)(i1 - i0) + (size_t)S + 1)); RC_TRY(dalloc(c, &orderN_out, (size_t)NN + 1));
    c->d_s2_order = c->d_s2_orderN = nullptr; c->n_s2_order = c->n_s2_orderN = 0;
    PoolScope s2_scope(c);
    const bool want_digest = P.stream_digest != 0;
    unsigned long long *d_digest = nullptr;
    c->have_digest = false;
    if (want_digest) { RC_TRY(dalloc(c, &d_digest, 4)); HIP_TRY(hipMemsetAsync(d_digest, 0, 32, c->stream)); }

    uint64_t *cand3 = nullptr; uint32_t *cand_order = nullptr; unsigned long long *best = nullptr;
    RC_TRY(dalloc(c, &cand3, (size_t)T * W3 + 1)); RC_TRY(dalloc(c, &cand_order, (size_t)T + 1)); RC_TRY(dalloc(c, &best, (size_t)T + 1));
    if (S) {
        if (c->d_sreads) hipLaunchKernelGGL(k_cand3_from2, G256((size_t)S * W3), c->d_sreads, (const uint32_t *)nullptr, S, L, W, W3, cand3);
        else hipLaunchKernelGGL(k_cand3_from2, G256((size_t)S * W3), c->d_reads, c->d_order_s, S, L, W, W3, cand3);
    }
    if (NN) HIP_TRY(hipMemcpyAsync(cand3 + (size_t)S * W3, c->d_nreads3, (size_t)NN * W3 * 8, hipMemcpyDeviceToDevice, c->stream));
    if (T) hipLaunchKernelGGL(k_cand_order, G256(T), c->d_order_s, S, T, cand_order);
    HIP_TRY(hipMemsetAsync(best, 0xFF, ((size_t)T + 1) * 8, c->stream));
    a.cand3 = cand3; a.cand_order = cand_order; a.best = best;
    uint8_t *head = nullptr; uint32_t *u1 = nullptr; uint64_t *gstart = nullptr; uint32_t *chead = nullptr;
    RC_TRY(dalloc(c, &head, (size_t)M + 1)); RC_TRY(dalloc(c, &u1, (size_t)M + 1)); RC_TRY(dalloc(c, &gstart, (size_t)M + 1));
    uint32_t nC = 0; uint64_t total = 0;
    if (M) {
        PoolScope cscope(c);
        uint32_t *u0 = nullptr; uint64_t *d64 = nullptr;
        RC_TRY(dalloc(c, &u0, (size_t)M + 1)); RC_TRY(dalloc(c, &d64, (size_t)M + 1));
        hipLaunchKernelGGL(k_heads1, G256(M), c->d_flag, M, a.q, head, u0);
        RC_TRY(prim_incl_max_u32(c, u0, u1, M));
        hipLaunchKernelGGL(k_heads2, G256(M), M, head, u1, u0);
        RC_TRY(prim_excl_scan_u32(c, u0, u1, M));
        hipLaunchKernelGGL(k_col_steps, G256(M), head, c->d_pos, M, L, d64);
        RC_TRY(prim_incl_scan_u64(c, d64, gstart, M));
        uint32_t lastcid = 0, lasthead = 0; uint64_t lastg = 0;
        HIP_TRY(hipMemcpyAsync(&lastcid, u1 + (M - 1), 4, hipMemcpyDeviceToHost, c->stream));
        HIP_TRY(hipMemcpyAsync(&lasthead, u0 + (M - 1), 4, hipMemcpyDeviceToHost, c->stream));
        HIP_TRY(hipMemcpyAsync(&lastg, gstart + (M - 1), 8, hipMemcpyDeviceToHost, c->stream));
        HIP_TRY(hipStreamSynchronize(c->stream));
        nC = lastcid + lasthead; total = lastg + (uint64_t)L;
    }
    RC_TRY(dalloc(c, &chead, (size_t)nC + 1));
    if (M) hipLaunchKernelGGL(k_contig_heads, G256(M), head, u1, M, chead);
    a.head = head; a.gstart = gstart; a.chead = chead; a.nC = nC; a.total = total;
    c->C.contigs = nC; c->C.seq_bases = total;
    std::vector<uint64_t> sh_col(E + 1, total), seq_off(E, 0), seq_nb(E, 0), seq_tl(E, 0);
    for (uint32_t e = 0; e <= E; e++) {
        const uint64_t st = (uint64_t)e * a.q; const uint32_t i = e == E ? M : (uint32_t)(st > M ? M : st);
        if (i >= M) { sh_col[e] = total; continue; }
        HIP_TRY(hipMemcpyAsync(&sh_col[e], gstart + i, 8, hipMemcpyDeviceToHost, c->stream));
    }
    HIP_TRY(hipStreamSynchronize(c->stream));
    const uint64_t col0 = sh_col[e0], col1 = sh_col[e1];
    a.col0 = col0; a.col1 = col1; a.tile_base = (uint32_t)(col0 / CTILE);
    if (part) c->C.seq_bases = col1 - col0;
    lap("contig structure (all reads, on every rank)");
    uint64_t *cons2 = nullptr;
    const uint64_t ncw = (total + 31) / 32;
    RC_TRY(dalloc(c, &cons2, (size_t)ncw + 2 * W + 4));
    HIP_TRY(hipMemsetAsync(cons2 + ncw, 0, ((size_t)2 * W + 4) * 8, c->stream));
    a.cons2 = cons2;
    uint64_t seq_total = 0;
    for (uint32_t e = e0; e < e1; e++) { const uint64_t cc = sh_col[e + 1] - sh_col[e]; seq_nb[e] = cc / 4; seq_tl[e] = cc % 4; seq_off[e] = seq_total; seq_total += (seq_nb[e] + seq_tl[e] + 15) & ~15ull; }
    uint8_t *seqpk = nullptr; RC_TRY(dalloc(c, &seqpk, (size_t)seq_total + 64));
    PoolScope ascope(c);
    uint64_t *cand2 = nullptr, *candN = nullptr;
    RC_TRY(dalloc(c, &cand2, (size_t)T * W + 1)); RC_TRY(dalloc(c, &candN, (size_t)T * W + 1));
    if (T) hipLaunchKernelGGL(k_cand2_from3, G256((size_t)T * W), (const uint64_t *)cand3, T, L, W, W3, cand2, candN);
    a.cand2 = cand2; a.candN = candN;
    a.maxevents = 1u << 20;
    if (c->s2_events_hint > a.maxevents) a.maxevents = c->s2_events_hint;
    if (const char *e = getenv("HARC_AMD_MAXEVENTS")) { a.maxevents = (uint32_t)strtoul(e, nullptr, 10); if (a.maxevents < 1) a.maxevents = 1; }
    RC_TRY(dalloc(c, &a.events, (size_t)a.maxevents)); RC_TRY(dalloc(c, &a.nevents, 4));
    HIP_TRY(hipMemsetAsync(a.nevents, 0, 16, c->stream));

    lap("  candidates: 3-bit store, 2-bit copies");
    DictDev dict[2];
    unsigned long long *d_big = nullptr; RC_TRY(dalloc(c, &d_big, 1));
    HIP_TRY(hipMemsetAsync(d_big, 0, 8, c->stream));
    uint32_t *bloom[2] = { nullptr, nullptr }; int bloom_shift[2] = { 63, 63 };
    const bool bloom4 = a.kbits[0] == a.kbits[1] && !getenv("HARC_AMD_BLOOM1");
    bool bloom4_tiled = false;
    int bloom_per_key = 16;
    if (const char *e = getenv("HARC_AMD_BLOOMBITS")) { bloom_per_key = atoi(e); if (bloom_per_key < 1) bloom_per_key = 1; }
    if (T) {
        RC_TRY(harc_dict_alloc(c, &dict[0], T, 0)); RC_TRY(harc_dict_alloc(c, &dict[1], T, dict[0].cap));
        dict[0].bigthresh = dict[1].bigthresh = (uint32_t)P.maxsearch < 32u ? (uint32_t)P.maxsearch : 32u;
        int lb = 16; while (lb < 36 && (1ULL << lb) < (unsigned long long)bloom_per_key * T) lb++;
        if (bloom4) {
            RC_TRY(dalloc(c, &bloom[0], ((size_t)1 << (lb - 3)) + 1));
            bloom4_tiled = getenv("HARC_AMD_S2BLOOM_TILED") ? atoi(getenv("HARC_AMD_S2BLOOM_TILED")) != 0 : (((size_t)1 << (lb - 3)) * 4 >= ((size_t)64 << 20));
            if ((uint64_t)T * 4 > 0xFFFFFFFFull || harc_bitmap_tiles((uint64_t)1 << (lb - 3)) + 1 >= (1u << BL_PART_BITS)) bloom4_tiled = false;
            if (!bloom4_tiled) HIP_TRY(hipMemsetAsync(bloom[0], 0, ((size_t)1 << (lb - 3)) * 4, c->stream));
            bloom[1] = bloom[0]; bloom_shift[0] = bloom_shift[1] = 64 - lb;
            a.bloom_lbits = lb - 7;
            a.bloom_nwin = (a.kbits[0] / 3 == 21 && !getenv("HARC_AMD_BLOOM4_HASHED")) ? 21 - BLOOM4_M + 1 : 0;
        } else for (int l = 0; l < 2; l++) {
            RC_TRY(dalloc(c, &bloom[l], ((size_t)1 << (lb - 5)) + 1));
            HIP_TRY(hipMemsetAsync(bloom[l], 0, ((size_t)1 << (lb - 5)) * 4, c->stream));
            bloom_shift[l] = 64 - lb;
        }
        PoolScope kscope(c);
        uint64_t *k0 = nullptr; uint32_t *i0k = nullptr; uint64_t *items = nullptr, *items_tmp = nullptr;
        RC_TRY(dalloc(c, &k0, T)); RC_TRY(dalloc(c, &i0k, T));
        const uint64_t b4words = (uint64_t)1 << (lb - 3);
        if (bloom4 && bloom4_tiled) { RC_TRY(dalloc(c, &items, (size_t)T * 4 + 1)); RC_TRY(dalloc(c, &items_tmp, (size_t)T * 4 + 1)); }
        for (int l = 0; l < 2; l++) {
            hipLaunchKernelGGL(k_key3, G256(T), cand3, T, W3, 3 * a.ds[l], a.kbits[l], k0, i0k);
            if (bloom4 && bloom4_tiled) hipLaunchKernelGGL(k_bloom4_items, G256(T), (const uint64_t *)k0, T, a.bloom_lbits, a.bloom_nwin, l, a.kbits[l] / 3, harc_bitmap_tiles(b4words), items + (size_t)l * 2 * T);
            else if (bloom4) hipLaunchKernelGGL(k_bloom4_set, G256(T), (const uint64_t *)k0, T, bloom[0], a.bloom_lbits, a.bloom_nwin, l, a.kbits[l] / 3);
            else hipLaunchKernelGGL(k_bloom_set, G256(T), (const uint64_t *)k0, T, bloom[l], bloom_shift[l]);
            lap("  keys, bitmap items");
            RC_TRY(harc_dict_build(c, &dict[l], k0, i0k, T, (unsigned)a.kbits[l], HARC_KEYS_RAW));
            hipLaunchKernelGGL(k_count_big_bins, G256(dict[l].cap), dict[l].slots, dict[l].cap, (uint32_t)P.maxsearch, d_big);
            lap("  dictionary built");
        }
        if (bloom4 && bloom4_tiled) {
            RC_TRY(harc_bitmap_from_items(c, items, items_tmp, (size_t)T * 4, b4words, bloom[0]));
            lap("  combined bitmap from sorted items");
            if (getenv("HARC_AMD_S2BLOOM_VERIFY")) {
                uint32_t *ref = nullptr; unsigned long long *nd = nullptr, hnd = 0;
                RC_TRY(dalloc(c, &ref, (size_t)b4words + 1)); RC_TRY(dalloc(c, &nd, 1));
                HIP_TRY(hipMemsetAsync(ref, 0, (size_t)b4words * 4, c->stream)); HIP_TRY(hipMemsetAsync(nd, 0, 8, c->stream));
                for (int l = 0; l < 2; l++) {
                    hipLaunchKernelGGL(k_key3, G256(T), cand3, T, W3, 3 * a.ds[l], a.kbits[l], k0, i0k);
                    hipLaunchKernelGGL(k_bloom4_set, G256(T), (const uint64_t *)k0, T, ref, a.bloom_lbits, a.bloom_nwin, l, a.kbits[l] / 3);
                }
                hipLaunchKernelGGL(k_words_differ, harc_grid256(b4words), dim3(256), 0, c->stream, (const uint32_t *)ref, (const uint32_t *)bloom[0], b4words, nd);
                HIP_TRY(hipMemcpyAsync(&hnd, nd, 8, hipMemcpyDeviceToHost, c->stream));
                HIP_TRY(hipStreamSynchronize(c->stream));
                if (hnd) { harc_set_error("stage II bitmap built by tiles differs from the one built with atomics in %llu words", hnd); return HARC_AMD_EINTERNAL; }
            }
        }
        HIP_TRY(hipStreamSynchronize(c->stream));
    }
    for (int l = 0; l < 2; l++) { a.slots[l] = dict[l].slots; a.cap[l] = dict[l].cap; a.ids[l] = dict[l].ids; a.bloom[l] = bloom[l]; a.bloom_shift[l] = bloom_shift[l]; }
    lap("candidates and their dictionaries (all candidates, on every rank)");

    uint8_t *h_seq = nullptr;
    struct CopyJoin { hipStream_t s; ~CopyJoin() { (void)hipStreamSynchronize(s); } } copy_join{ c->copy_stream };
    uint8_t *cons = nullptr; RC_TRY(dalloc(c, &cons, (size_t)total + 8));
    a.cons = cons;
    unsigned int nev = 0;
    if (col1 > col0) {
        unsigned long long *cinfo = nullptr; RC_TRY(dalloc(c, &cinfo, (size_t)nC + 1));
        hipLaunchKernelGGL(k_contig_info, G256(nC), a, cinfo);
        const uint32_t ntiles = (uint32_t)((col1 + CTILE - 1) / CTILE) - a.tile_base;
        uint32_t *tlo = nullptr, *thi = nullptr; RC_TRY(dalloc(c, &tlo, (size_t)ntiles + 1)); RC_TRY(dalloc(c, &thi, (size_t)ntiles + 1));
        hipLaunchKernelGGL(k_consensus_tiles, G256(ntiles), a, ntiles, tlo, thi);
        uint32_t *tovf = nullptr; RC_TRY(dalloc(c, &tovf, (size_t)ntiles + 1));
        HIP_TRY(hipMemsetAsync(tovf, 0, (size_t)ntiles * 4, c->stream));
        hipLaunchKernelGGL(k_consensus<CSHALLOW>, dim3(ntiles), dim3(CTHREADS), (size_t)CCHUNK * (W * 8 + 4), c->stream, a, (const uint32_t *)u1, (const unsigned long long *)cinfo, T ? 1 : 0,
                           (const uint32_t *)tlo, (const uint32_t *)thi, tovf);
        hipLaunchKernelGGL(k_consensus<CPLANES>, dim3(ntiles), dim3(CTHREADS), (size_t)CCHUNK * (W * 8 + 4), c->stream, a, (const uint32_t *)u1, (const unsigned long long *)cinfo, T ? 1 : 0,
                           (const uint32_t *)tlo, (const uint32_t *)thi, tovf);
        { const uint64_t w0 = col0 / 32, w1 = (col1 + 31) / 32; hipLaunchKernelGGL(k_pack_cons2, G256(w1 - w0), (const uint8_t *)a.cons, total, w0, w1 - w0, cons2); }
        {
            const uint64_t soff = seq_total;
            for (uint32_t e = e0; e < e1; e++) {
                const uint64_t cc0 = sh_col[e];
                if (seq_nb[e]) hipLaunchKernelGGL(k_pack2_bytes, G256(seq_nb[e]), cons + cc0, seq_nb[e], seqpk + seq_off[e]);
                if (seq_tl[e]) hipLaunchKernelGGL(k_bases_to_ascii, G256(seq_tl[e]), cons + cc0 + 4 * seq_nb[e], seq_tl[e], seqpk + seq_off[e] + seq_nb[e]);
            }
            HIP_TRY(hipGetLastError());
            if (want_digest) for (uint32_t e = e0; e < e1; e++) RC_TRY(digest_range(c, seqpk + seq_off[e], seq_nb[e] + seq_tl[e], 0x100 + e, d_digest + 0));
            RC_TRY(harc_host_alloc(c, (void **)&h_seq, (size_t)soff));
            HIP_TRY(hipEventRecord(c->ev_copy, c->stream));
            HIP_TRY(hipStreamWaitEvent(c->copy_stream, c->ev_copy, 0));
            if (soff) HIP_TRY(hipMemcpyAsync(h_seq, seqpk, (size_t)soff, hipMemcpyDeviceToHost, c->copy_stream));
        }
        if (T) {
            const dim3 rg(ntiles);
            auto propose = [&]() {
                switch (W) {
#define REALIGN_CASE(WW) case WW: if (bloom4 && a.bloom_nwin) hipLaunchKernelGGL((k_realign_propose1<WW, 21 - BLOOM4_M + 1>), rg, dim3(256), 0, c->stream, a); \
                                 else if (bloom4) hipLaunchKernelGGL((k_realign_propose1<WW, 0>), rg, dim3(256), 0, c->stream, a); \
                                 else hipLaunchKernelGGL((k_realign_propose<WW>), rg, dim3(256), 0, c->stream, a); break;
                    REALIGN_CASE(1) REALIGN_CASE(2) REALIGN_CASE(3) REALIGN_CASE(4) REALIGN_CASE(5) REALIGN_CASE(6) REALIGN_CASE(7) REALIGN_CASE(8)
#undef REALIGN_CASE
                }
            };
            propose();
            HIP_TRY(hipMemcpyAsync(&nev, a.nevents, 4, hipMemcpyDeviceToHost, c->stream));
            HIP_TRY(hipStreamSynchronize(c->stream));
            { const uint64_t want = (uint64_t)nev + nev / 4; c->s2_events_hint = want > 0xFFFFFFFFull ? 0xFFFFFFFFu : (uint32_t)want; }
            if (nev > a.maxevents) {
                a.maxevents = nev;
                RC_TRY(dalloc(c, &a.events, (size_t)a.maxevents));
                HIP_TRY(hipMemsetAsync(a.nevents, 0, 16, c->stream));
                propose();
                HIP_TRY(hipMemcpyAsync(&nev, a.nevents, 4, hipMemcpyDeviceToHost, c->stream));
                HIP_TRY(hipStreamSynchronize(c->stream));
                if (nev > a.maxevents) { harc_set_error("stage II: event count changed between two identical passes (%u > %u)", nev, a.maxevents); return HARC_AMD_EINTERNAL; }
            }
        }
    }
    HIP_TRY(hipGetLastError());
    unsigned long long *d_bdig = nullptr;
    auto best_digest = [&](const char *what) -> int {
        if (!getenv("HARC_AMD_TRACE") || !T) return HARC_AMD_OK;
        if (!d_bdig) RC_TRY(dalloc(c, &d_bdig, 2));
        unsigned long long hv = 0;
        HIP_TRY(hipMemsetAsync(d_bdig, 0, 8, c->stream));
        RC_TRY(digest_range(c, best, (uint64_t)T * 8, 0xBE57ull, d_bdig));
        HIP_TRY(hipMemcpyAsync(&hv, d_bdig, 8, hipMemcpyDeviceToHost, c->stream));
        HIP_TRY(hipStreamSynchronize(c->stream));
        fprintf(stderr, "[stage II] digest of the claims %s: %016llx (%u probes into large bins)\n", what, hv, nev);
        return HARC_AMD_OK;
    };
    RC_TRY(best_digest("after the proposals"));
    lap("consensus + read_seq + proposals (this rank's columns)");
    uint64_t *evwin = nullptr;
    if (nev) {
        RC_TRY(dalloc(c, &evwin, (size_t)nev * W3 + 1));
        WAVE_PER_ITEM(nev, hipLaunchKernelGGL(k_ev_windows, dim3(nb_), dim3(256), 0, c->stream, a, (const uint4 *)a.events, nev, evwin, kb_));
    }
    if (cm && T) {
        RC_TRY(cm->allreduce_min_u64(c, best, (size_t)T));
        RC_TRY(cm->wait(c, "all-reduce of the singleton / N-read claims"));
        std::vector<uint64_t> allnev((size_t)cm->world);
        { const uint64_t mine = nev; RC_TRY(cm->allgather_u64(c, &mine, 1, allnev.data())); }
        uint64_t tot = 0; for (uint64_t x : allnev) tot += x;
        if (tot > 0xFFFFFFFFull) { harc_set_error("stage II: more than 2^32 probes into large bins"); return HARC_AMD_EINVAL; }
        if (tot) {
            uint4 *ev_all = nullptr; uint64_t *win_all = nullptr;
            RC_TRY(dalloc(c, &ev_all, (size_t)tot + 1)); RC_TRY(dalloc(c, &win_all, (size_t)tot * W3 + 1));
            std::vector<size_t> so[2], sb[2], ro[2], rb[2];
            for (int k = 0; k < 2; k++) { so[k].assign(cm->world, 0); sb[k].resize(cm->world); ro[k].resize(cm->world); rb[k].resize(cm->world); }
            uint64_t acc = 0;
            for (int p = 0; p < cm->world; p++) {
                sb[0][p] = (size_t)nev * 16; sb[1][p] = (size_t)nev * W3 * 8;
                ro[0][p] = (size_t)acc * 16; rb[0][p] = (size_t)allnev[p] * 16; ro[1][p] = (size_t)acc * W3 * 8; rb[1][p] = (size_t)allnev[p] * W3 * 8;
                acc += allnev[p];
            }
            const void *sp[2] = { a.events, evwin }; void *rp[2] = { ev_all, win_all };
            const size_t *sop[2] = { so[0].data(), so[1].data() }, *sbp[2] = { sb[0].data(), sb[1].data() }, *rop[2] = { ro[0].data(), ro[1].data() }, *rbp[2] = { rb[0].data(), rb[1].data() };
            RC_TRY(cm->alltoallv(c, 2, sp, sop, sbp, rp, rop, rbp));
            RC_TRY(cm->wait(c, "all-gather of the probes into large bins"));
            a.events = ev_all; evwin = win_all; nev = (unsigned int)tot;
        } else nev = 0;
    }
    a.evwin = evwin;
    lap("all-reduce of the claims, probes into large bins gathered");
    if (nev) {
        unsigned int *d_changed = nullptr; uint32_t *estart = nullptr, *lastver = nullptr; unsigned long long *binmin[2] = { nullptr, nullptr };
        if (total >> (EV_TBITS - 2)) { harc_set_error("stage II: more than 2^%d consensus columns", EV_TBITS - 2); return HARC_AMD_EINVAL; }
// ... 92 lines not shown
            if (trace) { HIP_TRY(hipMemcpyAsync(&nlook, d_changed + 2, 4, hipMemcpyDeviceToHost, c->stream)); HIP_TRY(hipMemcpyAsync(&nwaves, d_changed + 3, 4, hipMemcpyDeviceToHost, c->stream)); HIP_TRY(hipMemcpyAsync(&nclaim, d_changed + 4, 4, hipMemcpyDeviceToHost, c->stream)); }
            HIP_TRY(hipStreamSynchronize(c->stream));
            if (trace) { struct timespec tw; clock_gettime(CLOCK_MONOTONIC, &tw); fprintf(stderr, "[stage II] window pass %llu over %u events (%u looked in %u waves, %u of them moved a claim), ranks [%u, %u)%s: %s, %.2f ms since the first\n", (unsigned long long)npass, nev, nlook, nwaves, nclaim, ranges ? rlo : 0u, ranges ? rhi : maxrank + 1, ranges ? "" : " (all)", chg ? "claims moved" : "quiet", (tw.tv_sec - tw0.tv_sec) * 1e3 + (tw.tv_nsec - tw0.tv_nsec) * 1e-6); }
            if (++npass > (uint64_t)T + 256) { harc_set_error("stage II: the window passes over the large bins did not settle"); return HARC_AMD_EINTERNAL; }
            if (chg && (!ranges || rhi <= pipeline_from)) continue;
            if (!ranges && !chg) break;
            if (!ranges) continue;
            if (rhi > maxrank) ranges = false;
            else { rlo = rhi; rhi = rhi > 0x20000000u ? 0xFFFFFFFFu : rhi * 4; ridx++; }
        }
    }
    HIP_TRY(hipGetLastError());

    RC_TRY(best_digest("after the window passes"));
    lap("window passes over the large bins (all probes, on every rank)");
    unsigned long long big = 0;
    HIP_TRY(hipMemcpyAsync(&big, d_big, 8, hipMemcpyDeviceToHost, c->stream));
    HIP_TRY(hipStreamSynchronize(c->stream));
    ascope.release_now();
    const uint32_t nt = t1 - t0;
    uint32_t *ls = nullptr, *ln = nullptr, *rs = nullptr, *rn = nullptr;
    RC_TRY(dalloc(c, &ls, (size_t)nt + 1)); RC_TRY(dalloc(c, &ln, (size_t)nt + 1)); RC_TRY(dalloc(c, &rs, (size_t)nt + 1)); RC_TRY(dalloc(c, &rn, (size_t)nt + 1));
    HIP_TRY(hipMemsetAsync(ls, 0, ((size_t)nt + 1) * 4, c->stream)); HIP_TRY(hipMemsetAsync(ln, 0, ((size_t)nt + 1) * 4, c->stream));
    if (nt) hipLaunchKernelGGL(k_left_flags, G256(nt), best, t0, nt, S, ls, ln);
    RC_TRY(prim_excl_scan_u32(c, ls, rs, (size_t)nt + 1)); RC_TRY(prim_excl_scan_u32(c, ln, rn, (size_t)nt + 1));
    uint32_t US = 0, UN = 0;
    HIP_TRY(hipMemcpyAsync(&US, rs + nt, 4, hipMemcpyDeviceToHost, c->stream));
    HIP_TRY(hipMemcpyAsync(&UN, rn + nt, 4, hipMemcpyDeviceToHost, c->stream));
    HIP_TRY(hipStreamSynchronize(c->stream));
    uint8_t *sing_bases = nullptr, *spk = nullptr; char *ntext = nullptr;
    const uint64_t sing_nb = (uint64_t)US * L / 4, sing_tl = (uint64_t)US * L % 4;
    const size_t n_ntext = (size_t)UN * (L + 1);
    RC_TRY(dalloc(c, &sing_bases, (size_t)US * L + 8)); RC_TRY(dalloc(c, &ntext, n_ntext + 1)); RC_TRY(dalloc(c, &spk, (size_t)(sing_nb + sing_tl) + 64));
    uint8_t *h_sing = nullptr, *h_ntext = nullptr;
    RC_TRY(harc_host_alloc(c, (void **)&h_sing, (size_t)(sing_nb + sing_tl))); RC_TRY(harc_host_alloc(c, (void **)&h_ntext, n_ntext));
    if (getenv("HARC_AMD_LEFT_ALL")) { if (nt) hipLaunchKernelGGL(k_left_emit, G256((uint64_t)nt * ((L + 15) / 16)), a, t0, nt, rs, rn, sing_bases, ntext); }
    else if (US + UN) {
        uint32_t *llist = nullptr;
        RC_TRY(dalloc(c, &llist, (size_t)US + UN + 1));
        hipLaunchKernelGGL(k_left_list, G256(nt), (const uint32_t *)ls, (const uint32_t *)ln, (const uint32_t *)rs, (const uint32_t *)rn, nt, US, llist);
        WAVE_PER_ITEM(US + UN, hipLaunchKernelGGL(k_left_emit_w, dim3(nb_), dim3(256), 0, c->stream, a, t0, (const uint32_t *)llist, US + UN, US, sing_bases, ntext, kb_));
    }
    if (sing_nb) hipLaunchKernelGGL(k_pack2_bytes, G256(sing_nb), sing_bases, sing_nb, spk);
    if (sing_tl) hipLaunchKernelGGL(k_bases_to_ascii, G256(sing_tl), sing_bases + 4 * sing_nb, sing_tl, spk + sing_nb);
    HIP_TRY(hipGetLastError());
    HIP_TRY(hipEventRecord(c->ev_copy, c->stream));
    HIP_TRY(hipStreamWaitEvent(c->copy_stream, c->ev_copy, 0));
    if (sing_nb + sing_tl) HIP_TRY(hipMemcpyAsync(h_sing, spk, (size_t)(sing_nb + sing_tl), hipMemcpyDeviceToHost, c->copy_stream));
    if (n_ntext) HIP_TRY(hipMemcpyAsync(h_ntext, ntext, n_ntext, hipMemcpyDeviceToHost, c->copy_stream));
    uint32_t A = 0;
    uint32_t *ta = nullptr, *tb = nullptr; uint64_t *tup0 = nullptr, *tup = nullptr; uint32_t *rid0 = nullptr, *rid = nullptr;
    RC_TRY(dalloc(c, &ta, (size_t)T + 1)); RC_TRY(dalloc(c, &tb, (size_t)T + 1));
    if (T) {
        HIP_TRY(hipMemsetAsync(ta, 0, ((size_t)T + 1) * 4, c->stream));
        hipLaunchKernelGGL(k_acc_flags, G256(T), best, T, ta);
        RC_TRY(prim_excl_scan_u32(c, ta, tb, (size_t)T + 1));
        HIP_TRY(hipMemcpyAsync(&A, tb + T, 4, hipMemcpyDeviceToHost, c->stream));
        HIP_TRY(hipStreamSynchronize(c->stream));
    }
    RC_TRY(dalloc(c, &tup0, (size_t)A + 1)); RC_TRY(dalloc(c, &tup, (size_t)A + 1)); RC_TRY(dalloc(c, &rid0, (size_t)A + 1)); RC_TRY(dalloc(c, &rid, (size_t)A + 1));
    if (A) {
        hipLaunchKernelGGL(k_acc_compact, G256(T), best, tb, T, A, tup0, rid0);
        unsigned bits = 2; while (bits < 64 && (total >> (bits - 2)) != 0) bits++;
        RC_TRY(prim_sort_pairs_u64_u32(c, tup0, tup, rid0, rid, A, bits));
    }

    lap("accepted candidates sorted (all, on every rank)");
    std::vector<uint32_t> sh_f(E + 1), sh_a(E + 1);
    {
        uint32_t *d_shf = nullptr, *d_sha = nullptr; uint64_t *d_shc = nullptr;
        RC_TRY(dalloc(c, &d_shf, (size_t)E + 2)); RC_TRY(dalloc(c, &d_sha, (size_t)E + 2)); RC_TRY(dalloc(c, &d_shc, (size_t)E + 2));
        hipLaunchKernelGGL(k_shard_bounds, G256(E + 1), (const uint64_t *)gstart, M, a.q, E, (const uint64_t *)tup, A, total, d_shf, d_sha, d_shc);
        HIP_TRY(hipMemcpyAsync(sh_f.data(), d_shf, ((size_t)E + 1) * 4, hipMemcpyDeviceToHost, c->stream));
        HIP_TRY(hipMemcpyAsync(sh_a.data(), d_sha, ((size_t)E + 1) * 4, hipMemcpyDeviceToHost, c->stream));
        HIP_TRY(hipStreamSynchronize(c->stream));
    }
    const uint32_t fbase = sh_f[e0], fend = sh_f[e1], F = fend - fbase, na = sh_a[e1] - sh_a[e0];
    if ((uint64_t)(i1 - i0) + na != F) { harc_set_error("stage II bookkeeping: %u reads + %u accepted candidates in a piece of %u", i1 - i0, na, F); return HARC_AMD_EINTERNAL; }

    FinalArrays f;
    RC_TRY(dalloc(c, &f.ref, (size_t)F + 1)); RC_TRY(dalloc(c, &f.kind, (size_t)F + 1)); RC_TRY(dalloc(c, &f.g, (size_t)F + 1));
    uint32_t *nm = nullptr, *nonN = nullptr, *nonNrank = nullptr; uint64_t *nmoff = nullptr;
    RC_TRY(dalloc(c, &nm, (size_t)F + 1)); RC_TRY(dalloc(c, &nonN, (size_t)F + 1)); RC_TRY(dalloc(c, &nonNrank, (size_t)F + 1)); RC_TRY(dalloc(c, &nmoff, (size_t)F + 1));
    HIP_TRY(hipMemsetAsync(nm, 0, ((size_t)F + 1) * 4, c->stream)); HIP_TRY(hipMemsetAsync(nonN, 0, ((size_t)F + 1) * 4, c->stream));
    uint8_t *posb = nullptr, *rcb = nullptr;
    RC_TRY(dalloc(c, &posb, (size_t)F + 1)); RC_TRY(dalloc(c, &rcb, (size_t)F + 8));
    uint8_t *h_packed = nullptr, *h_pos = nullptr, *h_meta = nullptr;
    RC_TRY(harc_host_alloc(c, (void **)&h_pos, F)); RC_TRY(harc_host_alloc(c, (void **)&h_meta, 32));
    unsigned long long *h_tot = nullptr; RC_TRY(harc_host_alloc(c, (void **)&h_tot, 16 * ((size_t)E + 2)));
    std::vector<uint64_t> sh_nm(E + 1, 0);
    std::vector<uint8_t *> g_noise(E, nullptr), g_noisepos(E, nullptr), gh_noise(E, nullptr), gh_noisepos(E, nullptr);
    std::vector<uint32_t> g_of(E, 0);
    std::vector<uint64_t> gtot(E, 0);
    std::vector<uint64_t> s_nz0(E, 0), s_nz1(E, 0), s_np0(E, 0), s_np1(E, 0);
    long long *mcut = nullptr; RC_TRY(dalloc(c, &mcut, (size_t)(i1 - i0) / 256 + 4));
    uint64_t nmtot = 0; uint32_t n_nonN = 0, n_N_aligned = 0;
    const uint32_t estep = (uint64_t)F * 3 >= ((uint64_t)32 << 20) ? 1u : (e1 - e0 ? e1 - e0 : 1u);
    for (uint32_t ea = e0; ea < e1; ea += estep) {
        const uint32_t eb = ea + estep < e1 ? ea + estep : e1;
        for (uint32_t e = ea; e < eb; e++) g_of[e] = ea;
        const uint32_t fa = sh_f[ea] - fbase, fb = sh_f[eb] - fbase;
        if (fb <= fa) continue;
        const uint32_t ia = (uint32_t)((uint64_t)ea * a.q > M ? M : (uint64_t)ea * a.q), ib = eb >= E ? M : (uint32_t)((uint64_t)eb * a.q > M ? M : (uint64_t)eb * a.q);
        if (ib > ia) {
            hipLaunchKernelGGL(k_merge_cuts, G256((ib - ia + 255u) / 256u + 1u), gstart, ia, ib - ia, tup, A, mcut);
            hipLaunchKernelGGL(k_merge_orig, G256(ib - ia), gstart, ia, ib - ia, tup, A, f, fbase, (const long long *)mcut);
        }
        if (sh_a[eb] > sh_a[ea]) hipLaunchKernelGGL(k_merge_acc, G256(sh_a[eb] - sh_a[ea]), gstart, M, tup, rid, sh_a[ea], sh_a[eb] - sh_a[ea], f, fbase);
        launch_noise<false>(c, a, f, cons2, fa, fb, nm, nonN, nullptr, nullptr, nullptr, nullptr, nullptr, nullptr, nullptr, nullptr);
        RC_TRY(prim_excl_scan_u32_to_u64(c, nm + fa, nmoff + fa, (size_t)(fb - fa) + 1));
        RC_TRY(prim_excl_scan_u32(c, nonN + fa, nonNrank + fa, (size_t)(fb - fa) + 1));
        HIP_TRY(hipMemcpyAsync(&h_tot[0], nmoff + fb, 8, hipMemcpyDeviceToHost, c->stream));
        HIP_TRY(hipMemcpyAsync(reinterpret_cast<uint32_t *>(&h_tot[1]), nonNrank + fb, 4, hipMemcpyDeviceToHost, c->stream));
        for (uint32_t e = ea + 1; e < eb; e++) HIP_TRY(hipMemcpyAsync(&h_tot[2 + (e - ea)], nmoff + (sh_f[e] - fbase), 8, hipMemcpyDeviceToHost, c->stream));
        HIP_TRY(hipStreamSynchronize(c->stream));
        const uint64_t gnm = h_tot[0]; const uint32_t gnon = *reinterpret_cast<uint32_t *>(&h_tot[1]), gF = fb - fa;
        sh_nm[ea] = 0; for (uint32_t e = ea + 1; e < eb; e++) sh_nm[e] = h_tot[2 + (e - ea)];
        RC_TRY(dalloc(c, &g_noise[ea], (size_t)gnm + gF + 8)); RC_TRY(dalloc(c, &g_noisepos[ea], (size_t)gnm + 8));
        RC_TRY(harc_host_alloc(c, (void **)&gh_noise[ea], (size_t)gnm + gF)); RC_TRY(harc_host_alloc(c, (void **)&gh_noisepos[ea], (size_t)gnm));
        launch_noise<true>(c, a, f, cons2, fa, fb, nullptr, nullptr, nmoff, nonNrank, g_noise[ea] - fa, g_noisepos[ea], posb, rcb, order_out + n_nonN, orderN_out + n_N_aligned - fa);
        HIP_TRY(hipEventRecord(c->ev_copy, c->stream));
        HIP_TRY(hipStreamWaitEvent(c->copy_stream, c->ev_copy, 0));
        if (gnm + gF) HIP_TRY(hipMemcpyAsync(gh_noise[ea], g_noise[ea], (size_t)gnm + gF, hipMemcpyDeviceToHost, c->copy_stream));
        if (gnm) HIP_TRY(hipMemcpyAsync(gh_noisepos[ea], g_noisepos[ea], (size_t)gnm, hipMemcpyDeviceToHost, c->copy_stream));
        HIP_TRY(hipMemcpyAsync(h_pos + fa, posb + fa, (size_t)gF, hipMemcpyDeviceToHost, c->copy_stream));
        nmtot += gnm; n_nonN += gnon; n_N_aligned += gF - gnon;
        gtot[ea] = gnm;
        for (uint32_t e = ea; e < eb; e++) {
            const uint64_t n0 = sh_nm[e], n1 = e + 1 < eb ? sh_nm[e + 1] : gnm;
            s_np0[e] = n0; s_np1[e] = n1; s_nz0[e] = n0 + (sh_f[e] - sh_f[ea]); s_nz1[e] = n1 + (sh_f[e + 1] - sh_f[ea]);
        }
    }
    if ((size_t)n_nonN + US > (size_t)(i1 - i0) + (size_t)S || (size_t)n_N_aligned + UN > (size_t)NN) { harc_set_error("stage II bookkeeping: %u + %u clean, %u + %u N order entries", n_nonN, US, n_N_aligned, UN); return HARC_AMD_EINTERNAL; }
    const size_t n_order = ((size_t)n_nonN + US) * 4, n_orderN = ((size_t)n_N_aligned + UN) * 4;
    if (nt) hipLaunchKernelGGL(k_left_orders, G256(nt), a, t0, nt, rs, rn, order_out, n_nonN, orderN_out, n_N_aligned);
    HIP_TRY(hipGetLastError());
    if (c->d_gid && !c->s1_from_files) {
        unsigned int *d_merr = nullptr; RC_TRY(dalloc(c, &d_merr, 4));
        HIP_TRY(hipMemsetAsync(d_merr, 0, 16, c->stream));
        RC_TRY(shard_map_ids(c, order_out, (uint64_t)n_nonN + US, c->d_gid, c->N, d_merr));
        RC_TRY(shard_map_ids(c, orderN_out, (uint64_t)n_N_aligned + UN, c->d_ngid, c->NN, d_merr));
        unsigned int merr = 0;
        HIP_TRY(hipMemcpyAsync(&merr, d_merr, 4, hipMemcpyDeviceToHost, c->stream));
        HIP_TRY(hipStreamSynchronize(c->stream));
        if (merr) { harc_set_error("stage II: %u order entries outside the shard", merr); return HARC_AMD_EINTERNAL; }
    }

    std::vector<uint64_t> rev_off(E, 0), rev_nb(E, 0), rev_tl(E, 0);
    uint64_t poff = 0;
    for (uint32_t e = e0; e < e1; e++) {
        const uint64_t ff = sh_f[e + 1] - sh_f[e]; rev_nb[e] = ff / 8; rev_tl[e] = ff % 8; rev_off[e] = poff; poff += (rev_nb[e] + rev_tl[e] + 15) & ~15ull;
    }
    uint8_t *packed = nullptr; RC_TRY(dalloc(c, &packed, (size_t)poff + 64));
    for (uint32_t e = e0; e < e1; e++) {
        const uint32_t f0 = sh_f[e] - fbase;
        if (rev_nb[e]) hipLaunchKernelGGL(k_pack1_bytes, G256(rev_nb[e]), rcb + f0, rev_nb[e], packed + rev_off[e]);
        if (rev_tl[e]) HIP_TRY(hipMemcpyAsync(packed + rev_off[e] + rev_nb[e], rcb + f0 + 8 * rev_nb[e], rev_tl[e], hipMemcpyDeviceToDevice, c->stream));
    }
    HIP_TRY(hipGetLastError());
    RC_TRY(harc_host_alloc(c, (void **)&h_packed, (size_t)poff));
    HIP_TRY(hipEventRecord(c->ev_copy, c->stream));
    HIP_TRY(hipStreamWaitEvent(c->copy_stream, c->ev_copy, 0));
    if (poff) HIP_TRY(hipMemcpyAsync(h_packed, packed, (size_t)poff, hipMemcpyDeviceToHost, c->copy_stream));
    if (want_digest) {
        for (uint32_t e = e0; e < e1; e++) if (g_of[e] == e && g_noise[e]) {
            uint32_t eb = e; while (eb < e1 && g_of[eb] == e) eb++;
            RC_TRY(digest_range(c, g_noise[e], gtot[e] + (sh_f[eb] - sh_f[e]), 0x200 + 16 * e, d_digest + 1)); RC_TRY(digest_range(c, g_noisepos[e], gtot[e], 0x201 + 16 * e, d_digest + 1));
// ... 68 lines not shown
```

include/harc_amd.h:

```cpp
#ifndef HARC_AMD_H
#define HARC_AMD_H
#include <stddef.h>
#include <stdint.h>

#ifdef __cplusplus
extern "C" {
#endif

#define HARC_AMD_OK 0
#define HARC_AMD_EINVAL (-1)
#define HARC_AMD_ENODEVICE (-2)
#define HARC_AMD_EIO (-3)
#define HARC_AMD_ESTATE (-4)
#define HARC_AMD_ENOMEM (-5)
#define HARC_AMD_ETIMEOUT (-7)
#define HARC_AMD_EINTERNAL (-6)

typedef struct harc_amd_params {
    int32_t readlen;
    int32_t num_thr;
    int32_t num_chains;
    int32_t maxmatch;
    int32_t thresh;
    int32_t thresh_s;
// ... 34 lines not shown

enum {
    HARC_AMD_S1_ORDER = 0,
    HARC_AMD_S1_FLAG = 1,
    HARC_AMD_S1_POS = 2,
    HARC_AMD_S1_RC = 3,
    HARC_AMD_S1_ORDER_SINGLETON = 4,
    HARC_AMD_S1_DNA = 5,
    HARC_AMD_S1_DNA_SINGLETON = 6,
    HARC_AMD_S2_SEQ = 10,
    HARC_AMD_S2_SEQ_TAIL = 11,
    HARC_AMD_S2_POS = 12,
    HARC_AMD_S2_NOISE = 13,
    HARC_AMD_S2_NOISEPOS = 14,
    HARC_AMD_S2_REV = 15,
    HARC_AMD_S2_REV_TAIL = 16,
    HARC_AMD_S2_ORDER = 20,
    HARC_AMD_S2_ORDER_N_PE = 21,
    HARC_AMD_S2_SINGLETON = 22,
    HARC_AMD_S2_SINGLETON_TAIL = 23,
    HARC_AMD_S2_INPUT_N = 24,
    HARC_AMD_S2_META = 25,
    HARC_AMD_P_ORDER = 30,
    HARC_AMD_P_ORDER_TAIL = 31,
    HARC_AMD_IN_ORDER_N = 40
};

typedef struct harc_amd_ctx harc_amd_ctx;

int harc_amd_default_params(int32_t readlen, harc_amd_params *out);

int harc_amd_create(const harc_amd_params *params, harc_amd_ctx **out);
void harc_amd_destroy(harc_amd_ctx *ctx);
const char *harc_amd_last_error(void);

int harc_amd_set_reads_ascii(harc_amd_ctx *ctx, const char *ascii, uint32_t n_reads, uint32_t stride);
int harc_amd_set_reads_ascii_device(harc_amd_ctx *ctx, const char *d_ascii, uint32_t n_reads, uint32_t stride);
int harc_amd_set_reads_packed_device(harc_amd_ctx *ctx, const uint64_t *d_packed, uint32_t n_reads);
int harc_amd_set_nreads_ascii(harc_amd_ctx *ctx, const char *ascii, uint32_t n_reads, uint32_t stride);
int harc_amd_set_nreads_ascii_device(harc_amd_ctx *ctx, const char *d_ascii, uint32_t n_reads, uint32_t stride);
int harc_amd_set_fastq_device(harc_amd_ctx *ctx, const char *d_fastq, uint64_t n_bytes, uint64_t *n_records_out);
int harc_amd_bgzf_inflate_device(harc_amd_ctx *ctx, const uint8_t *d_bgzf, uint64_t n_bytes, char *d_out, uint64_t out_capacity, uint64_t *n_out);
uint64_t harc_amd_bgzf_bound(uint64_t n_text);
int harc_amd_bgzf_deflate_device(harc_amd_ctx *ctx, const char *d_text, uint64_t n_bytes, int32_t flags, uint8_t *d_out, uint64_t out_capacity, uint64_t *n_out);
int harc_amd_bgzf_deflate_host(const char *text, uint64_t n_bytes, int32_t flags, uint8_t *out, uint64_t out_capacity, uint64_t *n_out);
int harc_amd_fastq_assemble_device(harc_amd_ctx *ctx, const char *d_ids, uint64_t id_bytes, const char *d_dna, const char *d_quality, uint32_t n_records,
                                   int32_t readlen, char *d_out, uint64_t out_capacity, uint64_t *n_out);
int harc_amd_set_fastq_bgzf_device(harc_amd_ctx *ctx, const uint8_t *d_bgzf, uint64_t n_bytes, uint64_t *n_records_out);
int harc_amd_set_stage1_streams(harc_amd_ctx *ctx, const char *temp_dna, const uint8_t *flag, const uint8_t *pos,
                                const uint32_t *order, const uint8_t *rc, uint32_t n_main,
                                const char *temp_dna_singleton, const uint32_t *order_singleton, uint32_t n_singleton);

int harc_amd_pack_reads_device(harc_amd_ctx *ctx, const char *d_ascii, uint32_t n_reads, uint32_t stride, uint64_t *d_packed_out);
int harc_amd_bucket_reads_device(harc_amd_ctx *ctx, const uint64_t *d_packed, uint32_t n_reads, uint32_t n_buckets, uint32_t *d_bucket_out);
int harc_amd_partition_reads_device(harc_amd_ctx *ctx, const uint64_t *d_packed, uint32_t n_reads, uint32_t n_buckets, uint64_t *d_packed_out, uint64_t *d_counts_out);

#define HARC_AMD_COMM_ID_BYTES 128
int harc_amd_comm_get_id(uint8_t *id, size_t id_bytes);
int harc_amd_comm_init(harc_amd_ctx *ctx, const uint8_t *id, size_t id_bytes, int32_t world, int32_t rank);
int harc_amd_comm_init_mailbox(harc_amd_ctx *ctx, const char *dir, int32_t world, int32_t rank);
int harc_amd_comm_barrier(harc_amd_ctx *ctx);
int harc_amd_comm_destroy(harc_amd_ctx *ctx);
int harc_amd_shard_exchange(harc_amd_ctx *ctx, uint64_t *info);
int harc_amd_replicate_exchange(harc_amd_ctx *ctx, uint64_t *info);
int harc_amd_shard_reset(harc_amd_ctx *ctx);

int harc_amd_reorder(harc_amd_ctx *ctx);
int harc_amd_encode(harc_amd_ctx *ctx);
int harc_amd_pack_order(harc_amd_ctx *ctx);

int harc_amd_get_stream(harc_amd_ctx *ctx, int32_t stream_id, int32_t shard, const void **ptr, size_t *len);
int harc_amd_get_counters(harc_amd_ctx *ctx, harc_amd_counters *out);

int harc_amd_decode_signature(harc_amd_ctx *ctx, uint64_t sig[3]);
int harc_amd_reads_signature_device(harc_amd_ctx *ctx, const char *d_ascii, uint32_t n_reads, uint32_t stride, uint64_t sig[3]);
int harc_amd_input_signature(harc_amd_ctx *ctx, uint64_t sig[3]);

int harc_amd_stream_digest(harc_amd_ctx *ctx, uint64_t out[4]);
const char *harc_amd_build_id(void);
int harc_amd_build_has(const char *feature);
int harc_amd_selftest_launch(harc_amd_ctx *ctx, uint64_t n, uint64_t *visited, uint64_t *index_sum);
int harc_amd_selftest_index(harc_amd_ctx *ctx, const uint64_t *keys, uint64_t n, int32_t slots_per_read, uint32_t bigthresh, int32_t want_large,
                            uint64_t *cap, uint32_t *nbins, void *slots, uint32_t *ids, uint64_t *large, uint64_t large_capacity, uint64_t *n_large);

int harc_amd_last_fastq_timing(double *out, int32_t n);

int harc_amd_reorder_files(const harc_amd_params *params, const char *basedir);
int harc_amd_encoder_files(const harc_amd_params *params, const char *basedir);
int harc_amd_compress_files(const harc_amd_params *params, const char *basedir);
int harc_amd_pack_order_files(const harc_amd_params *params, const char *basedir);
int harc_amd_compress_fastq_files(const harc_amd_params *params, const char *fastq, const char *basedir);
int harc_amd_compress_fastq_files_ex(const harc_amd_params *params, const char *fastq, const char *basedir, int32_t preserve_order, int32_t preserve_quality);
int harc_amd_fastq_assemble_files(const harc_amd_params *params, const char *dna_path, const char *id_path, const char *quality_path, const char *out_path);
int harc_amd_fastq_assemble_files_ex(const harc_amd_params *params, const char *dna_path, const char *id_path, const char *quality_path, const char *out_path, int32_t bgzf);
int harc_amd_preprocess_files(const char *fastq, const char *basedir, int32_t readlen);
int harc_amd_decoder_files(const harc_amd_params *params, const char *basedir, int32_t num_thr_e);
int harc_amd_decoder_preserve_files(const harc_amd_params *params, const char *basedir, int32_t num_thr_e);
int harc_amd_compress_fastq_shard_files(const harc_amd_params *params, const char *fastq, const char *basedir, int32_t preserve_order,
                                        int32_t preserve_quality, int32_t world, int32_t rank, const char *comm_spec);
int harc_amd_merge_shard_files(const char *basedir, int32_t world);
int harc_amd_compress_fastq_replicated_files(const harc_amd_params *params, const char *fastq, const char *basedir, int32_t preserve_order,
                                             int32_t preserve_quality, int32_t world, int32_t rank, const char *comm_spec);

uint64_t harc_amd_qpack_bound(uint64_t n_reads, int32_t readlen, uint32_t reads_per_block);
int harc_amd_qpack_device(harc_amd_ctx *ctx, const char *d_text, uint64_t n_reads, int32_t readlen, uint32_t reads_per_block, int32_t flags, uint8_t *d_out,
                          uint64_t out_capacity, uint64_t *n_out);
int harc_amd_qunpack_device(harc_amd_ctx *ctx, const uint8_t *d_packed, uint64_t n_bytes, char *d_text, uint64_t out_capacity, uint64_t *n_out);
int harc_amd_qpack_host(const char *text, uint64_t n_reads, int32_t readlen, uint32_t reads_per_block, int32_t flags, uint8_t *out, uint64_t cap, uint64_t *n_out);
int harc_amd_qunpack_host(const uint8_t *packed, uint64_t n_bytes, char *text, uint64_t cap, uint64_t *n_out);
int harc_amd_qpack_files(const harc_amd_params *params, const char *quality_path, const char *out_path);
int harc_amd_qunpack_files(const harc_amd_params *params, const char *packed_path, const char *out_path);

typedef struct harc_amd_qmap {
    int32_t kind;
    int32_t radius;
    uint8_t table[256];
} harc_amd_qmap;
typedef struct harc_amd_qmap_stats {
    uint64_t values;
    uint64_t changed;
    uint64_t sum_abs;
    uint64_t sum_sq;
    uint32_t max_abs;
    uint32_t distinct_in;
    uint32_t distinct_out;
    uint32_t reserved;
} harc_amd_qmap_stats;
int harc_amd_qmap_parse(const char *spec, harc_amd_qmap *out);
int harc_amd_qmap_host(const char *text, uint64_t n_reads, int32_t readlen, const harc_amd_qmap *map, char *out, harc_amd_qmap_stats *stats);
int harc_amd_qmap_device(harc_amd_ctx *ctx, const char *d_text, uint64_t n_reads, int32_t readlen, const harc_amd_qmap *map, char *d_out, harc_amd_qmap_stats *stats);
int harc_amd_qmap_files(const harc_amd_params *params, const char *quality_path, const char *out_path, const harc_amd_qmap *map, harc_amd_qmap_stats *stats);
int harc_amd_qpack_files_ex(const harc_amd_params *params, const char *quality_path, const char *out_path, const harc_amd_qmap *map, harc_amd_qmap_stats *stats);

#define HARC_AMD_IDPACK_NO_HEADER 1
uint64_t harc_amd_idpack_bound(uint64_t text_bytes, uint64_t n_lines, uint32_t lines_per_block);
int harc_amd_idpack_device(harc_amd_ctx *ctx, const char *d_text, uint64_t text_bytes, uint32_t lines_per_block, int32_t flags, uint8_t *d_out, uint64_t out_capacity,
                           uint64_t *n_out);
int harc_amd_idunpack_device(harc_amd_ctx *ctx, const uint8_t *d_packed, uint64_t n_bytes, char *d_text, uint64_t out_capacity, uint64_t *n_out);
int harc_amd_idpack_host(const char *text, uint64_t text_bytes, uint32_t lines_per_block, int32_t flags, uint8_t *out, uint64_t cap, uint64_t *n_out);
int harc_amd_idunpack_host(const uint8_t *packed, uint64_t n_bytes, char *text, uint64_t cap, uint64_t *n_out);
int harc_amd_idpack_files(const harc_amd_params *params, const char *id_path, const char *out_path);
int harc_amd_idunpack_files(const harc_amd_params *params, const char *packed_path, const char *out_path);

uint64_t harc_amd_spack_bound(uint64_t text_bytes, uint32_t block_bytes);
int harc_amd_spack_device(harc_amd_ctx *ctx, const uint8_t *d_text, uint64_t text_bytes, uint32_t block_bytes, int32_t flags, uint8_t *d_out, uint64_t out_capacity,
                          uint64_t *n_out);
int harc_amd_sunpack_device(harc_amd_ctx *ctx, const uint8_t *d_packed, uint64_t n_bytes, uint8_t *d_text, uint64_t out_capacity, uint64_t *n_out);
int harc_amd_spack_host(const uint8_t *text, uint64_t text_bytes, uint32_t block_bytes, int32_t flags, uint8_t *out, uint64_t cap, uint64_t *n_out);
int harc_amd_sunpack_host(const uint8_t *packed, uint64_t n_bytes, uint8_t *text, uint64_t cap, uint64_t *n_out);
int harc_amd_spack_files(const harc_amd_params *params, const char *in_path, const char *out_path);
int harc_amd_sunpack_files(const harc_amd_params *params, const char *packed_path, const char *out_path);
int harc_amd_spack_file_list(const harc_amd_params *params, int32_t n_files, const char *const *in_paths, const char *const *out_paths);
int harc_amd_sunpack_file_list(const harc_amd_params *params, int32_t n_files, const char *const *packed_paths, const char *const *out_paths);

int harc_amd_text_digest_device(harc_amd_ctx *ctx, const void *d_text, uint64_t nbytes, uint64_t first_offset, uint64_t acc[3]);
int harc_amd_text_digest_host(const void *text, uint64_t nbytes, uint64_t first_offset, uint64_t acc[3]);
int harc_amd_text_digest_files(const harc_amd_params *params, const char *path, uint64_t out[3]);
int harc_amd_input_order_digest(harc_amd_ctx *ctx, uint64_t out[3]);
int harc_amd_reads_check_files(const harc_amd_params *params, const char *dna_path, uint64_t sig[3], uint64_t t[3]);
int harc_amd_compress_fastq_files_checked(const harc_amd_params *params, const char *fastq, const char *basedir, int32_t preserve_order, int32_t preserve_quality, int32_t check);

#ifdef __cplusplus
}
#endif
#endif
```

Measured before the change: 743.0.

## Fuse contig structure scan, pack cons2 in consensus, compact overflow tiles

Replaces the multi-pass contig head and offset computation (max-scan, exclusive scan, step scan, and several small device-to-host copies) with a single two-pass decoupled segment scan that also emits shard column starts. The consensus kernel now writes the 2-bit packed cons2 words directly, which removes the separate pack kernel. Per-shard sequence packing collapses into one 2D launch that reads cons2. The deep consensus pass only visits the tiles that overflowed, through a compacted list in a persistent grid. It also drops a few memsets and adds a pool shrink call. The aim is fewer launches, host syncs and memory passes, at the cost of more complex code and a new selftest entry point.

```diff
diff --git a/harc_amd/api.py b/harc_amd/api.py
--- a/harc_amd/api.py
+++ b/harc_amd/api.py
@@ -154,6 +154,9 @@
     l.harc_amd_selftest_launch.argtypes = [ctx, C.c_uint64, C.POINTER(C.c_uint64), C.POINTER(C.c_uint64)]
     l.harc_amd_selftest_index.argtypes = [ctx, C.c_void_p, C.c_uint64, C.c_int32, C.c_uint32, C.c_int32, C.POINTER(C.c_uint64), C.POINTER(C.c_uint32), C.c_void_p, C.c_void_p,
                                           C.c_void_p, C.c_uint64, C.POINTER(C.c_uint64)]
+    if hasattr(l, "harc_amd_selftest_contigs"):
+        l.harc_amd_selftest_contigs.argtypes = [ctx, C.c_void_p, C.c_void_p, C.c_uint64, C.c_int32, C.c_uint32, C.c_uint32, C.c_void_p, C.c_void_p, C.c_void_p, C.c_void_p,
+                                                C.POINTER(C.c_uint32), C.POINTER(C.c_uint64), C.POINTER(C.c_int32)]
     U3 = C.POINTER(C.c_uint64)
     l.harc_amd_text_digest_device.argtypes = [ctx, C.c_void_p, C.c_uint64, C.c_uint64, U3]
     l.harc_amd_text_digest_host.argtypes = [C.c_char_p, C.c_uint64, C.c_uint64, U3]
@@ -632,6 +635,21 @@
             raise HarcAmdError(-1, "harc_amd_selftest_index lists %d large bins among %d keys" % (nl.value, n))
         return int(cap.value), int(nbins.value), slots, ids, (large[:nl.value].copy() if want_large else None)
 
+    def selftest_contigs(self, flag, pos, L, q, cut=10000000):
+        import numpy as np
+        flag = np.ascontiguousarray(flag, dtype=np.uint8)
+        pos = np.ascontiguousarray(pos, dtype=np.uint8)
+        n = int(flag.size)
+        if int(pos.size) != n:
+            raise HarcAmdError(-1, "selftest_contigs: %d flags, %d positions" % (n, int(pos.size)))
+        head = np.zeros(n, dtype=np.uint8)
+        cid, chead = np.zeros(n, dtype=np.uint32), np.zeros(n, dtype=np.uint32)
+        gstart = np.zeros(n, dtype=np.uint64)
+        nc, total, fb = C.c_uint32(0), C.c_uint64(0), C.c_int32(0)
+        _check(lib().harc_amd_selftest_contigs(self._ctx, flag.ctypes.data, pos.ctypes.data, n, L, q, cut, head.ctypes.data, cid.ctypes.data, gstart.ctypes.data,
+                                               chead.ctypes.data, C.byref(nc), C.byref(total), C.byref(fb)))
+        return head, cid, gstart, chead[:nc.value].copy(), int(nc.value), int(total.value), bool(fb.value)
+
     def stream_digest(self):
         d = (C.c_uint64 * 4)()
         _check(lib().harc_amd_stream_digest(self._ctx, d))
diff --git a/harc_amd/csrc/api.cpp b/harc_amd/csrc/api.cpp
--- a/harc_amd/csrc/api.cpp
+++ b/harc_amd/csrc/api.cpp
@@ -91,6 +91,15 @@
     return HARC_AMD_OK;
 }
 void harc_dev_free(harc_amd_ctx *c, void *p) { (void)c; (void)p; }
+void harc_dev_shrink(harc_amd_ctx *c, void *p, size_t bytes)
+{
+    if (c->pool_cur >= c->pool.size()) return;
+    harc_amd_ctx::PoolChunk &k = c->pool[c->pool_cur];
+    bytes = (bytes + 255) & ~(size_t)255;
+    if (bytes == 0) bytes = 256;
+    if ((char *)p < k.base || (char *)p + bytes > k.base + k.used) return;
+    k.used = (size_t)((char *)p - k.base) + bytes;
+}
 harc_mark_t harc_pool_mark(harc_amd_ctx *c)
 {
     if (c->pool.empty()) return 0;
diff --git a/harc_amd/csrc/internal.h b/harc_amd/csrc/internal.h
--- a/harc_amd/csrc/internal.h
+++ b/harc_amd/csrc/internal.h
@@ -144,6 +144,8 @@
 int harc_dev_alloc(harc_amd_ctx *c, void **p, size_t bytes);
 void harc_dev_free(harc_amd_ctx *c, void *p);
 template <class T> static inline int dalloc(harc_amd_ctx *c, T **p, size_t n) { return harc_dev_alloc(c, (void **)p, n * sizeof(T) + 16); }
+void harc_dev_shrink(harc_amd_ctx *c, void *p, size_t bytes);
+template <class T> static inline void dshrink(harc_amd_ctx *c, T *p, size_t n) { harc_dev_shrink(c, (void *)p, n * sizeof(T) + 16); }
 int harc_tmp_reserve(harc_amd_ctx *c, size_t bytes);
 int harc_raw_alloc(harc_amd_ctx *c, void **p, size_t bytes);
 void harc_raw_free(harc_amd_ctx *c, void *p);
@@ -177,6 +179,8 @@
 int prim_incl_scan_u64(harc_amd_ctx *c, const uint64_t *in, uint64_t *out, size_t n);
 int prim_incl_max_u32(harc_amd_ctx *c, const uint32_t *in, uint32_t *out, size_t n);
 int prim_bins_scan(harc_amd_ctx *c, const uint64_t *skeys, size_t n, uint64_t cap, uint32_t *binstart, uint64_t *q, uint32_t *nbins, void *scratch, size_t scratch_bytes);
+int prim_contig_scan(harc_amd_ctx *c, const uint8_t *flag, const uint8_t *pos, size_t n, uint32_t L, uint32_t q, uint32_t cut, uint8_t *head, uint32_t *cid, uint64_t *gstart,
+                     uint32_t *chead, unsigned long long *info);
 
 int s1_pack_ascii(harc_amd_ctx *c, const char *d_ascii, uint32_t n, uint32_t stride, uint64_t *d_out);
 int s1_pack3_ascii(harc_amd_ctx *c, const char *d_ascii, uint32_t n, uint32_t stride, uint64_t *d_out);
diff --git a/harc_amd/csrc/prims.hip b/harc_amd/csrc/prims.hip
--- a/harc_amd/csrc/prims.hip
+++ b/harc_amd/csrc/prims.hip
@@ -143,6 +143,83 @@
     hipLaunchKernelGGL(k_bins_pass<false>, grid, dim3(256), 0, c->stream, skeys, (uint32_t)n, cap, (uint32_t)seg, nseg, part, (uint32_t *)nullptr, (uint64_t *)nullptr, (uint32_t *)nullptr);
     PRIM_CALL(rocprim::exclusive_scan(tmp, bytes, part, front, BinPart{ BINS_NONE, 0u, 0u }, (size_t)nseg, BinPartOp(), c->stream));
     hipLaunchKernelGGL(k_bins_pass<true>, grid, dim3(256), 0, c->stream, skeys, (uint32_t)n, cap, (uint32_t)seg, nseg, front, binstart, q, nbins);
+    HIP_TRY(hipGetLastError());
+    return HARC_AMD_OK;
+}
+
+struct ContigPart { uint64_t s; uint32_t c, last; };
+struct ContigPartOp {
+    __host__ __device__ ContigPart operator()(const ContigPart &a, const ContigPart &b) const { return ContigPart{ a.s + b.s, a.c + b.c, a.last > b.last ? a.last : b.last }; }
+};
+#define CONTIG_SEG_MIN 2048u
+#define CONTIG_SEGS 16384u
+#define CONTIG_UNROLL 4
+template <bool WRITE> __global__ __launch_bounds__(256) void k_contig_pass(const uint8_t *flag, const uint8_t *pos, uint32_t n, uint32_t L, uint32_t q, uint32_t cut, uint32_t seg, uint32_t nseg,
+                                                                         ContigPart *part, uint8_t *head, uint32_t *cid, uint64_t *gstart, uint32_t *chead, unsigned long long *info)
+{
+    const uint32_t w = (blockIdx.x * 256u + threadIdx.x) >> 6;
+    if (w >= nseg) return;
+    const uint32_t lane = threadIdx.x & 63;
+    const unsigned long long upto = ~0ull >> (63 - lane);
+    uint32_t C = 0, last = 0; uint64_t G = 0;
+    if (WRITE) { C = part[w].c; last = part[w].last; G = part[w].s; }
+    const uint64_t base = (uint64_t)w * seg, end = base + seg < n ? base + seg : (uint64_t)n;
+    uint32_t rem = (uint32_t)(base % q);
+    for (uint64_t at = base; at < end; at += 64u * CONTIG_UNROLL) {
+        uint8_t f[CONTIG_UNROLL], p[CONTIG_UNROLL];
+#pragma unroll
+        for (int u = 0; u < CONTIG_UNROLL; u++) { const uint64_t i = at + 64u * u + lane; f[u] = i < end ? flag[i] : (uint8_t)0; p[u] = i < end ? pos[i] : (uint8_t)0; }
+#pragma unroll
+        for (int u = 0; u < CONTIG_UNROLL; u++) {
+            const uint64_t i0 = at + 64u * u, i = i0 + lane;
+            const uint32_t m = rem + lane;
+            const bool sh = q >= 128u ? (m == 0 || m == q) : (m % q) == 0;
+            if (q >= 128u) { rem += 64u; if (rem >= q) rem -= q; } else rem = (rem + 64u) % q;
+            const bool h = i < end && (f[u] == '0' || sh);
+            const unsigned long long hb = __ballot(h);
+            uint32_t v = i >= end ? 0u : h ? (i == 0 ? 0u : L) : (uint32_t)p[u];
+            if (WRITE) {
+                const uint32_t rank = C + (uint32_t)__popcll(hb & upto) - (h ? 1u : 0u);
+                for (int d = 1; d < 64; d <<= 1) { const uint32_t o = __shfl_up(v, d, 64); if (lane >= (uint32_t)d) v += o; }
+                const uint64_t g = G + v;
+                const unsigned long long mine = hb & upto;
+                const uint32_t l1 = mine ? (uint32_t)i0 + 63u - (uint32_t)__clzll(mine) : last;
+                if (i < end) {
+                    head[i] = h ? 1 : 0; cid[i] = rank; gstart[i] = g;
+                    if (h) chead[rank] = (uint32_t)i;
+                    if (sh) info[3 + (uint32_t)i / q] = g;
+                    if ((uint32_t)i - l1 > cut) info[2] = 1;
+                    if (i + 1 == n) { info[0] = rank + (h ? 1u : 0u); info[1] = g + L; }
+                }
+                G += __shfl(v, 63, 64);
+            } else {
+                for (int o = 32; o > 0; o >>= 1) v += __shfl_xor(v, o, 64);
+                G += v;
+            }
+            if (hb) last = (uint32_t)i0 + 63u - (uint32_t)__clzll(hb);
+            C += (uint32_t)__popcll(hb);
+        }
+    }
+    if (!WRITE && lane == 0) part[w] = ContigPart{ G, C, last };
+}
+int prim_contig_scan(harc_amd_ctx *c, const uint8_t *flag, const uint8_t *pos, size_t n, uint32_t L, uint32_t q, uint32_t cut, uint8_t *head, uint32_t *cid, uint64_t *gstart,
+                     uint32_t *chead, unsigned long long *info)
+{
+    if (n == 0) return HARC_AMD_OK;
+    if (n > 0xFFFFFFFFull || q == 0) { harc_set_error("prim_contig_scan: %zu reads, shards of %u", n, q); return HARC_AMD_EINVAL; }
+    size_t seg = (n + CONTIG_SEGS - 1) / CONTIG_SEGS;
+    if (seg < CONTIG_SEG_MIN) seg = CONTIG_SEG_MIN;
+    seg = (seg + 64 * CONTIG_UNROLL - 1) / (64 * CONTIG_UNROLL) * (64 * CONTIG_UNROLL);
+    const uint32_t nseg = (uint32_t)((n + seg - 1) / seg);
+    PoolScope scope(c);
+    ContigPart *part = nullptr; RC_TRY(dalloc(c, &part, (size_t)2 * nseg));
+    ContigPart *front = part + nseg;
+    const dim3 grid((nseg + 3) / 4);
+    HIP_TRY(hipMemsetAsync(info + 2, 0, 8, c->stream));
+    hipLaunchKernelGGL(k_contig_pass<false>, grid, dim3(256), 0, c->stream, flag, pos, (uint32_t)n, L, q, cut, (uint32_t)seg, nseg, part, (uint8_t *)nullptr, (uint32_t *)nullptr, (uint64_t *)nullptr,
+                       (uint32_t *)nullptr, (unsigned long long *)nullptr);
+    PRIM_CALL(rocprim::exclusive_scan(tmp, bytes, part, front, ContigPart{ 0, 0u, 0u }, (size_t)nseg, ContigPartOp(), c->stream));
+    hipLaunchKernelGGL(k_contig_pass<true>, grid, dim3(256), 0, c->stream, flag, pos, (uint32_t)n, L, q, cut, (uint32_t)seg, nseg, front, head, cid, gstart, chead, info);
     HIP_TRY(hipGetLastError());
     return HARC_AMD_OK;
 }
diff --git a/harc_amd/csrc/stage2.hip b/harc_amd/csrc/stage2.hip
--- a/harc_amd/csrc/stage2.hip
+++ b/harc_amd/csrc/stage2.hip
@@ -24,7 +24,7 @@
     unsigned long long *bestbin[2];
     const uint32_t *bloom[2]; int bloom_shift[2];
     int bloom_lbits, bloom_nwin;
-    const uint64_t *cons2;
+    uint64_t *cons2;
     const uint64_t *cand2, *candN;
     uint4 *events;
     unsigned int *nevents; uint32_t maxevents;
@@ -107,12 +107,12 @@
     const uint8_t h = (flag[i] == '0' || (i % q) == 0) ? 1 : 0;
     head[i] = h; hidx[i] = h ? i : 0;
 }
-__global__ void k_heads2(uint32_t M, uint8_t *head, const uint32_t *hmax, uint32_t *hidx)
+__global__ void k_heads2(uint32_t M, uint32_t cut, uint8_t *head, const uint32_t *hmax, uint32_t *hidx)
 {
     const uint32_t i = harc_gid32();
     if (i >= M) return;
     const uint32_t r = i - hmax[i];
-    if (r > 0 && (r % 10000001u) == 0) head[i] = 1;
+    if (r > 0 && (r % (cut + 1u)) == 0) head[i] = 1;
     hidx[i] = head[i] ? 1u : 0u;
 }
 __global__ void k_col_steps(const uint8_t *head, const uint8_t *pos, uint32_t M, int L, uint64_t *d)
@@ -158,15 +158,14 @@
     thi[t] = (uint32_t)ub_le(s.gstart, (long long)s.M, X1 - 1);
     tlo[t] = X0 >= (uint64_t)s.L ? (uint32_t)(ub_le(s.gstart, (long long)s.M, X0 - (uint64_t)s.L) + 1) : 0u;
 }
-template <int NPL> __global__ __launch_bounds__(CTHREADS, NPL == CPLANES ? 4 : 6) void k_consensus(S2Args s, const uint32_t *cid, const unsigned long long *cinfo, int want_windows, const uint32_t *tlo, const uint32_t *thi, uint32_t *tovf)
-{
-    if (NPL == CPLANES && !tovf[blockIdx.x]) return;
+template <int NPL> __device__ __forceinline__ bool consensus_tile(const S2Args &s, const uint32_t tile, const uint32_t *cid, const unsigned long long *cinfo, int want_windows, const uint32_t *tlo, const uint32_t *thi)
+{
     extern __shared__ uint64_t cl_words[];
     int *const cl_g = reinterpret_cast<int *>(cl_words + (size_t)CCHUNK * s.W);
     const uint32_t *const cl_w32 = reinterpret_cast<const uint32_t *>(cl_words);
-    const uint64_t X0 = (uint64_t)(blockIdx.x + s.tile_base) * CTILE;
+    const uint64_t X0 = (uint64_t)(tile + s.tile_base) * CTILE;
     const int L = s.L, W = s.W;
-    const long long ilo = tlo[blockIdx.x], ihi = thi[blockIdx.x];
+    const long long ilo = tlo[tile], ihi = thi[tile];
     const int x0r = (int)threadIdx.x * CSTRIP;
     const uint64_t x0 = X0 + (uint64_t)x0r;
     const bool mine = x0 < s.total;
@@ -264,8 +263,11 @@
         }
     }
     flush();
-    if (NPL < CPLANES && ovf) tovf[blockIdx.x] = 1;
-    if (!mine) return;
+    uint32_t *const cons2h = reinterpret_cast<uint32_t *>(s.cons2);
+    if (!mine) {
+        if (x0 < ((s.total + 31) & ~31ull)) cons2h[x0 / CSTRIP] = 0;
+        return ovf;
+    }
     depth = __builtin_amdgcn_readfirstlane(depth);
     uint32_t lt = 0, dec = 0, lt2 = 0, dec2 = 0;
 #pragma unroll
@@ -278,6 +280,7 @@
             lt2 |= d & ~dec2 & (w >> 1); dec2 |= d;
         }
     const uint32_t indw = (lt2 & (lt >> 1)) | (~lt2 & lt & EVEN) | (lt2 << 1);
+    cons2h[x0 / CSTRIP] = (((indw & EVEN) << 1) | ((indw >> 1) & EVEN)) & (ncol == CSTRIP ? 0xFFFFFFFFu : (1u << (2 * ncol)) - 1u);
     uint32_t outw[CSTRIP / 4];
     uint32_t vmask = 0;
     if (want_windows) {
@@ -312,6 +315,17 @@
         *reinterpret_cast<uint4 *>(s.cons + x0) = make_uint4(outw[0], outw[1], outw[2], outw[3]);
     } else {
         for (int c = 0; c < ncol; c++) s.cons[x0 + c] = (uint8_t)(outw[c >> 2] >> (8 * (c & 3)));
+    }
+    return ovf;
+}
+template <int NPL> __global__ __launch_bounds__(CTHREADS, NPL == CPLANES ? 4 : 6) void k_consensus(S2Args s, const uint32_t *cid, const unsigned long long *cinfo, int want_windows, const uint32_t *tlo, const uint32_t *thi, uint32_t *tovf)
+{
+    if (NPL == CPLANES) {
+        const uint32_t n = tovf[0];
+        for (uint32_t k = blockIdx.x; k < n; k += gridDim.x) consensus_tile<NPL>(s, tovf[1 + k], cid, cinfo, want_windows, tlo, thi);
+    } else {
+        const bool ovf = consensus_tile<NPL>(s, blockIdx.x, cid, cinfo, want_windows, tlo, thi);
+        if (__syncthreads_or(ovf) && threadIdx.x == 0) tovf[1 + atomicAdd(&tovf[0], 1u)] = blockIdx.x;
     }
 }
 
@@ -1151,22 +1165,6 @@
     sh_f[e] = (uint32_t)st + (uint32_t)(lo + 1); sh_a[e] = (uint32_t)(lo + 1); sh_col[e] = g;
 }
 
-__global__ void k_pack_cons2(const uint8_t *cons, uint64_t total, uint64_t w0, uint64_t nwords, uint64_t *cons2)
-{
-    const uint64_t w = w0 + harc_gid();
-    if (w >= w0 + nwords) return;
-    uint64_t v = 0;
-    const uint64_t c0 = w * 32;
-    if (c0 + 32 <= total) {
-        const uint4 q0 = *(const uint4 *)(cons + c0), q1 = *(const uint4 *)(cons + c0 + 16);
-        const uint32_t qq[8] = { q0.x, q0.y, q0.z, q0.w, q1.x, q1.y, q1.z, q1.w };
-#pragma unroll
-        for (int k = 0; k < 32; k++) { const uint32_t idx = (qq[k >> 2] >> (8 * (k & 3))) & 3; v |= (uint64_t)(((idx & 1) << 1) | (idx >> 1)) << (2 * k); }
-    } else {
-        for (int k = 0; k < 32 && c0 + k < total; k++) { const uint32_t idx = cons[c0 + k] & 3; v |= (uint64_t)(((idx & 1) << 1) | (idx >> 1)) << (2 * k); }
-    }
-    cons2[w] = v;
-}
 template <int W> __device__ __forceinline__ void final_words(const S2Args &s, uint32_t ref, int kind, uint64_t (&rd)[W], uint64_t (&nmk)[W])
 {
     if (kind == 0) {
@@ -1226,6 +1224,7 @@
     if (!EMIT) {
         nm[i] = cnt;
         nonN[i] = (kind != 0 && ref >= s.S) ? 0u : 1u;
+        if (i + 1 == F) nm[F] = nonN[F] = 0;
         return;
     }
     uint64_t np = nmoff[i], nz = nmoff[i] + i;
@@ -1321,6 +1320,22 @@
     if (!single && lane == 0) ot[s.L] = '\n';
 }
 
+struct SeqShard { uint64_t col0, nbytes, off; };
+__global__ __launch_bounds__(256) void k_pack_seq(const uint64_t *cons2, const SeqShard *shards, uint8_t *out)
+{
+    const SeqShard sh = shards[blockIdx.y];
+    const uint64_t j = (uint64_t)blockIdx.x * 256u + threadIdx.x;
+    if (8 * j >= sh.nbytes) return;
+    const uint64_t x = sh.col0 + 32 * j;
+    const uint64_t *w = cons2 + (x >> 5);
+    const int b = 2 * (int)(x & 31);
+    uint64_t v = w[0] >> b;
+    if (b) v |= w[1] << (64 - b);
+    v = ((v & 0x5555555555555555ULL) << 1) | ((v >> 1) & 0x5555555555555555ULL);
+    uint8_t *o = out + sh.off + 8 * j;
+    if (8 * j + 8 <= sh.nbytes) *reinterpret_cast<uint64_t *>(o) = v;
+    else for (uint64_t k = 0; 8 * j + k < sh.nbytes; k++) o[k] = (uint8_t)(v >> (8 * k));
+}
 __global__ void k_pack2_bytes(const uint8_t *bases, uint64_t nbytes_out, uint8_t *out)
 {
     const uint64_t i = harc_gid();
@@ -1385,6 +1400,84 @@
     hipLaunchKernelGGL(k_stream_digest, dim3(nb), dim3(256), 0, c->stream, (const uint8_t *)base, nbytes, salt, d_out);
     HIP_TRY(hipGetLastError());
     return HARC_AMD_OK;
+}
+
+#define CONTIG_CUT 10000000u
+static int contig_structure(harc_amd_ctx *c, const uint8_t *flag, const uint8_t *pos, uint32_t M, int L, uint32_t q, uint32_t cut, uint32_t E, uint8_t *head, uint32_t *cid,
+                            uint64_t *gstart, uint32_t *chead, uint32_t *nC, uint64_t *total, uint64_t *sh_col, int *fellback)
+{
+    *nC = 0; *total = 0;
+    if (fellback) *fellback = 0;
+    for (uint32_t e = 0; e <= E; e++) sh_col[e] = 0;
+    if (!M) return HARC_AMD_OK;
+    PoolScope scope(c);
+    const uint32_t nsh = (M - 1u) / q + 1u;
+    std::vector<unsigned long long> hinfo((size_t)3 + nsh, 0);
+    unsigned long long *info = nullptr; RC_TRY(dalloc(c, &info, hinfo.size()));
+    RC_TRY(prim_contig_scan(c, flag, pos, M, (uint32_t)L, q, cut, head, cid, gstart, chead, info));
+    HIP_TRY(hipMemcpyAsync(hinfo.data(), info, hinfo.size() * 8, hipMemcpyDeviceToHost, c->stream));
+    HIP_TRY(hipStreamSynchronize(c->stream));
+    if (!hinfo[2]) {
+        *nC = (uint32_t)hinfo[0]; *total = hinfo[1];
+        for (uint32_t e = 0; e <= E; e++) sh_col[e] = e < nsh && e < E ? hinfo[3 + e] : *total;
+        return HARC_AMD_OK;
+    }
+    if (fellback) *fellback = 1;
+    uint32_t *u0 = nullptr; uint64_t *d64 = nullptr;
+    RC_TRY(dalloc(c, &u0, (size_t)M + 1)); RC_TRY(dalloc(c, &d64, (size_t)M + 1));
+    hipLaunchKernelGGL(k_heads1, G256(M), flag, M, q, head, u0);
+    RC_TRY(prim_incl_max_u32(c, u0, cid, M));
+    hipLaunchKernelGGL(k_heads2, G256(M), M, cut, head, cid, u0);
+    RC_TRY(prim_excl_scan_u32(c, u0, cid, M));
+    hipLaunchKernelGGL(k_col_steps, G256(M), head, pos, M, L, d64);
+    RC_TRY(prim_incl_scan_u64(c, d64, gstart, M));
+    hipLaunchKernelGGL(k_contig_heads, G256(M), head, cid, M, chead);
+    uint32_t lastcid = 0, lasthead = 0; uint64_t lastg = 0;
+    HIP_TRY(hipMemcpyAsync(&lastcid, cid + (M - 1), 4, hipMemcpyDeviceToHost, c->stream));
+    HIP_TRY(hipMemcpyAsync(&lasthead, u0 + (M - 1), 4, hipMemcpyDeviceToHost, c->stream));
+    HIP_TRY(hipMemcpyAsync(&lastg, gstart + (M - 1), 8, hipMemcpyDeviceToHost, c->stream));
+    for (uint32_t e = 0; e < E && e < nsh; e++) HIP_TRY(hipMemcpyAsync(&sh_col[e], gstart + (size_t)e * q, 8, hipMemcpyDeviceToHost, c->stream));
+    HIP_TRY(hipStreamSynchronize(c->stream));
+    *nC = lastcid + lasthead; *total = lastg + (uint64_t)L;
+    for (uint32_t e = 0; e <= E; e++) if (e >= nsh || e >= E) sh_col[e] = *total;
+    return HARC_AMD_OK;
+}
+
+static int selftest_contigs(harc_amd_ctx *c, const uint8_t *flag, const uint8_t *pos, uint32_t M, int L, uint32_t q, uint32_t cut, uint8_t *head, uint32_t *cid, uint64_t *gstart,
+                            uint32_t *chead, uint32_t *nC, uint64_t *total, int32_t *fellback)
+{
+    PoolScope scope(c);
+    uint8_t *d_flag = nullptr, *d_pos = nullptr, *d_head = nullptr; uint32_t *d_cid = nullptr, *d_chead = nullptr; uint64_t *d_gstart = nullptr;
+    RC_TRY(dalloc(c, &d_flag, M)); RC_TRY(dalloc(c, &d_pos, M)); RC_TRY(dalloc(c, &d_head, (size_t)M + 1)); RC_TRY(dalloc(c, &d_cid, (size_t)M + 1));
+    RC_TRY(dalloc(c, &d_gstart, (size_t)M + 1)); RC_TRY(dalloc(c, &d_chead, (size_t)M + 1));
+    HIP_TRY(hipMemcpyAsync(d_flag, flag, M, hipMemcpyHostToDevice, c->stream));
+    HIP_TRY(hipMemcpyAsync(d_pos, pos, M, hipMemcpyHostToDevice, c->stream));
+    HIP_TRY(hipMemsetAsync(d_head, 0xA5, M, c->stream)); HIP_TRY(hipMemsetAsync(d_cid, 0xA5, (size_t)M * 4, c->stream));
+    HIP_TRY(hipMemsetAsync(d_gstart, 0xA5, (size_t)M * 8, c->stream)); HIP_TRY(hipMemsetAsync(d_chead, 0xA5, (size_t)M * 4, c->stream));
+    const uint32_t E = (M - 1u) / q + 1u;
+    std::vector<uint64_t> sh_col((size_t)E + 1, 0);
+    int fb = 0;
+    RC_TRY(contig_structure(c, d_flag, d_pos, M, L, q, cut, E, d_head, d_cid, d_gstart, d_chead, nC, total, sh_col.data(), &fb));
+    *fellback = fb;
+    HIP_TRY(hipMemcpyAsync(head, d_head, M, hipMemcpyDeviceToHost, c->stream));
+    HIP_TRY(hipMemcpyAsync(cid, d_cid, (size_t)M * 4, hipMemcpyDeviceToHost, c->stream));
+    HIP_TRY(hipMemcpyAsync(gstart, d_gstart, (size_t)M * 8, hipMemcpyDeviceToHost, c->stream));
+    HIP_TRY(hipMemcpyAsync(chead, d_chead, (size_t)M * 4, hipMemcpyDeviceToHost, c->stream));
+    HIP_TRY(hipStreamSynchronize(c->stream));
+    for (uint32_t e = 0; e < E; e++)
+        if (sh_col[e] != gstart[(size_t)e * q]) { harc_set_error("harc_amd_selftest_contigs: shard %u starts at column %llu, its first read at %llu", e, (unsigned long long)sh_col[e], (unsigned long long)gstart[(size_t)e * q]); return HARC_AMD_EINTERNAL; }
+    if (sh_col[E] != *total) { harc_set_error("harc_amd_selftest_contigs: the column behind the last shard is not the total"); return HARC_AMD_EINTERNAL; }
+    return HARC_AMD_OK;
+}
+extern "C" int harc_amd_selftest_contigs(harc_amd_ctx *c, const uint8_t *flag, const uint8_t *pos, uint64_t n, int32_t readlen, uint32_t q, uint32_t cut, uint8_t *head, uint32_t *cid,
+                                         uint64_t *gstart, uint32_t *chead, uint32_t *ncontigs, uint64_t *total, int32_t *fellback)
+{
+    if (!c || !flag || !pos || n == 0 || n > 0xFFFFFFF0ull || readlen < 1 || readlen > 255 || q == 0 || cut == 0xFFFFFFFFu) { harc_set_error("harc_amd_selftest_contigs: bad arguments"); return HARC_AMD_EINVAL; }
+    if (!head || !cid || !gstart || !chead || !ncontigs || !total || !fellback) { harc_set_error("harc_amd_selftest_contigs: a NULL output"); return HARC_AMD_EINVAL; }
+    HIP_TRY(hipSetDevice(c->P.device));
+    const int rc = selftest_contigs(c, flag, pos, (uint32_t)n, readlen, q, cut, head, cid, gstart, chead, ncontigs, total, fellback);
+    if (rc != HARC_AMD_OK) (void)hipStreamSynchronize(c->stream);
+    return rc;
 }
 
 int stage2_run(harc_amd_ctx *c)
@@ -1434,35 +1527,13 @@
     a.cand3 = cand3; a.cand_order = cand_order; a.best = best;
     uint8_t *head = nullptr; uint32_t *u1 = nullptr; uint64_t *gstart = nullptr; uint32_t *chead = nullptr;
     RC_TRY(dalloc(c, &head, (size_t)M + 1)); RC_TRY(dalloc(c, &u1, (size_t)M + 1)); RC_TRY(dalloc(c, &gstart, (size_t)M + 1));
+    RC_TRY(dalloc(c, &chead, (size_t)M + 1));
     uint32_t nC = 0; uint64_t total = 0;
-    if (M) {
-        PoolScope cscope(c);
-        uint32_t *u0 = nullptr; uint64_t *d64 = nullptr;
-        RC_TRY(dalloc(c, &u0, (size_t)M + 1)); RC_TRY(dalloc(c, &d64, (size_t)M + 1));
-        hipLaunchKernelGGL(k_heads1, G256(M), c->d_flag, M, a.q, head, u0);
-        RC_TRY(prim_incl_max_u32(c, u0, u1, M));
-        hipLaunchKernelGGL(k_heads2, G256(M), M, head, u1, u0);
-        RC_TRY(prim_excl_scan_u32(c, u0, u1, M));
-        hipLaunchKernelGGL(k_col_steps, G256(M), head, c->d_pos, M, L, d64);
-        RC_TRY(prim_incl_scan_u64(c, d64, gstart, M));
-        uint32_t lastcid = 0, lasthead = 0; uint64_t lastg = 0;
-        HIP_TRY(hipMemcpyAsync(&lastcid, u1 + (M - 1), 4, hipMemcpyDeviceToHost, c->stream));
-        HIP_TRY(hipMemcpyAsync(&lasthead, u0 + (M - 1), 4, hipMemcpyDeviceToHost, c->stream));
-        HIP_TRY(hipMemcpyAsync(&lastg, gstart + (M - 1), 8, hipMemcpyDeviceToHost, c->stream));
-        HIP_TRY(hipStreamSynchronize(c->stream));
-        nC = lastcid + lasthead; total = lastg + (uint64_t)L;
-    }
-    RC_TRY(dalloc(c, &chead, (size_t)nC + 1));
-    if (M) hipLaunchKernelGGL(k_contig_heads, G256(M), head, u1, M, chead);
+    std::vector<uint64_t> sh_col(E + 1, 0), seq_off(E, 0), seq_nb(E, 0), seq_tl(E, 0);
+    RC_TRY(contig_structure(c, c->d_flag, c->d_pos, M, L, a.q, CONTIG_CUT, E, head, u1, gstart, chead, &nC, &total, sh_col.data(), nullptr));
+    dshrink(c, chead, (size_t)nC + 1);
     a.head = head; a.gstart = gstart; a.chead = chead; a.nC = nC; a.total = total;
     c->C.contigs = nC; c->C.seq_bases = total;
-    std::vector<uint64_t> sh_col(E + 1, total), seq_off(E, 0), seq_nb(E, 0), seq_tl(E, 0);
-    for (uint32_t e = 0; e <= E; e++) {
-        const uint64_t st = (uint64_t)e * a.q; const uint32_t i = e == E ? M : (uint32_t)(st > M ? M : st);
-        if (i >= M) { sh_col[e] = total; continue; }
-        HIP_TRY(hipMemcpyAsync(&sh_col[e], gstart + i, 8, hipMemcpyDeviceToHost, c->stream));
-    }
-    HIP_TRY(hipStreamSynchronize(c->stream));
     const uint64_t col0 = sh_col[e0], col1 = sh_col[e1];
     a.col0 = col0; a.col1 = col1; a.tile_base = (uint32_t)(col0 / CTILE);
     if (part) c->C.seq_bases = col1 - col0;
@@ -1475,6 +1546,7 @@
     uint64_t seq_total = 0;
     for (uint32_t e = e0; e < e1; e++) { const uint64_t cc = sh_col[e + 1] - sh_col[e]; seq_nb[e] = cc / 4; seq_tl[e] = cc % 4; seq_off[e] = seq_total; seq_total += (seq_nb[e] + seq_tl[e] + 15) & ~15ull; }
     uint8_t *seqpk = nullptr; RC_TRY(dalloc(c, &seqpk, (size_t)seq_total + 64));
+    std::vector<SeqShard> seq_shards(e1 - e0);
     PoolScope ascope(c);
     uint64_t *cand2 = nullptr, *candN = nullptr;
     RC_TRY(dalloc(c, &cand2, (size_t)T * W + 1)); RC_TRY(dalloc(c, &candN, (size_t)T * W + 1));
@@ -1561,19 +1633,24 @@
         uint32_t *tlo = nullptr, *thi = nullptr; RC_TRY(dalloc(c, &tlo, (size_t)ntiles + 1)); RC_TRY(dalloc(c, &thi, (size_t)ntiles + 1));
         hipLaunchKernelGGL(k_consensus_tiles, G256(ntiles), a, ntiles, tlo, thi);
         uint32_t *tovf = nullptr; RC_TRY(dalloc(c, &tovf, (size_t)ntiles + 1));
-        HIP_TRY(hipMemsetAsync(tovf, 0, (size_t)ntiles * 4, c->stream));
+        HIP_TRY(hipMemsetAsync(tovf, 0, 4, c->stream));
         hipLaunchKernelGGL(k_consensus<CSHALLOW>, dim3(ntiles), dim3(CTHREADS), (size_t)CCHUNK * (W * 8 + 4), c->stream, a, (const uint32_t *)u1, (const unsigned long long *)cinfo, T ? 1 : 0,
                            (const uint32_t *)tlo, (const uint32_t *)thi, tovf);
-        hipLaunchKernelGGL(k_consensus<CPLANES>, dim3(ntiles), dim3(CTHREADS), (size_t)CCHUNK * (W * 8 + 4), c->stream, a, (const uint32_t *)u1, (const unsigned long long *)cinfo, T ? 1 : 0,
+        hipLaunchKernelGGL(k_consensus<CPLANES>, dim3(ntiles < 1024u ? ntiles : 1024u), dim3(CTHREADS), (size_t)CCHUNK * (W * 8 + 4), c->stream, a, (const uint32_t *)u1, (const unsigned long long *)cinfo, T ? 1 : 0,
                            (const uint32_t *)tlo, (const uint32_t *)thi, tovf);
-        { const uint64_t w0 = col0 / 32, w1 = (col1 + 31) / 32; hipLaunchKernelGGL(k_pack_cons2, G256(w1 - w0), (const uint8_t *)a.cons, total, w0, w1 - w0, cons2); }
         {
             const uint64_t soff = seq_total;
-            for (uint32_t e = e0; e < e1; e++) {
-                const uint64_t cc0 = sh_col[e];
-                if (seq_nb[e]) hipLaunchKernelGGL(k_pack2_bytes, G256(seq_nb[e]), cons + cc0, seq_nb[e], seqpk + seq_off[e]);
-                if (seq_tl[e]) hipLaunchKernelGGL(k_bases_to_ascii, G256(seq_tl[e]), cons + cc0 + 4 * seq_nb[e], seq_tl[e], seqpk + seq_off[e] + seq_nb[e]);
+            uint64_t maxnb = 0;
+            for (uint32_t e = e0; e < e1; e++) { seq_shards[e - e0] = SeqShard{ sh_col[e], seq_nb[e], seq_off[e] }; if (seq_nb[e] > maxnb) maxnb = seq_nb[e]; }
+            if (maxnb) {
+                SeqShard *d_shards = nullptr; RC_TRY(dalloc(c, &d_shards, (size_t)(e1 - e0)));
+                HIP_TRY(hipMemcpyAsync(d_shards, seq_shards.data(), (size_t)(e1 - e0) * sizeof(SeqShard), hipMemcpyHostToDevice, c->stream));
+                for (uint32_t y = 0; y < e1 - e0; y += 65535u)
+                    hipLaunchKernelGGL(k_pack_seq, dim3((unsigned)((maxnb + 8 * 256 - 1) / (8 * 256)), e1 - e0 - y < 65535u ? e1 - e0 - y : 65535u), dim3(256), 0, c->stream, (const uint64_t *)cons2,
+                                       (const SeqShard *)d_shards + y, seqpk);
             }
+            for (uint32_t e = e0; e < e1; e++)
+                if (seq_tl[e]) hipLaunchKernelGGL(k_bases_to_ascii, G256(seq_tl[e]), cons + sh_col[e] + 4 * seq_nb[e], seq_tl[e], seqpk + seq_off[e] + seq_nb[e]);
             HIP_TRY(hipGetLastError());
             if (want_digest) for (uint32_t e = e0; e < e1; e++) RC_TRY(digest_range(c, seqpk + seq_off[e], seq_nb[e] + seq_tl[e], 0x100 + e, d_digest + 0));
             RC_TRY(harc_host_alloc(c, (void **)&h_seq, (size_t)soff));
@@ -1832,7 +1909,6 @@
     RC_TRY(dalloc(c, &f.ref, (size_t)F + 1)); RC_TRY(dalloc(c, &f.kind, (size_t)F + 1)); RC_TRY(dalloc(c, &f.g, (size_t)F + 1));
     uint32_t *nm = nullptr, *nonN = nullptr, *nonNrank = nullptr; uint64_t *nmoff = nullptr;
     RC_TRY(dalloc(c, &nm, (size_t)F + 1)); RC_TRY(dalloc(c, &nonN, (size_t)F + 1)); RC_TRY(dalloc(c, &nonNrank, (size_t)F + 1)); RC_TRY(dalloc(c, &nmoff, (size_t)F + 1));
-    HIP_TRY(hipMemsetAsync(nm, 0, ((size_t)F + 1) * 4, c->stream)); HIP_TRY(hipMemsetAsync(nonN, 0, ((size_t)F + 1) * 4, c->stream));
     uint8_t *posb = nullptr, *rcb = nullptr;
     RC_TRY(dalloc(c, &posb, (size_t)F + 1)); RC_TRY(dalloc(c, &rcb, (size_t)F + 8));
     uint8_t *h_packed = nullptr, *h_pos = nullptr, *h_meta = nullptr;
diff --git a/include/harc_amd.h b/include/harc_amd.h
--- a/include/harc_amd.h
+++ b/include/harc_amd.h
@@ -140,6 +140,8 @@
 int harc_amd_selftest_launch(harc_amd_ctx *ctx, uint64_t n, uint64_t *visited, uint64_t *index_sum);
 int harc_amd_selftest_index(harc_amd_ctx *ctx, const uint64_t *keys, uint64_t n, int32_t slots_per_read, uint32_t bigthresh, int32_t want_large,
                             uint64_t *cap, uint32_t *nbins, void *slots, uint32_t *ids, uint64_t *large, uint64_t large_capacity, uint64_t *n_large);
+int harc_amd_selftest_contigs(harc_amd_ctx *ctx, const uint8_t *flag, const uint8_t *pos, uint64_t n, int32_t readlen, uint32_t q, uint32_t cut, uint8_t *head, uint32_t *cid,
+                              uint64_t *gstart, uint32_t *chead, uint32_t *ncontigs, uint64_t *total, int32_t *fellback);
 
 int harc_amd_last_fastq_timing(double *out, int32_t n);
 
```

After: 757.8 (median of 6 runs). +2.0%, better.
